# SandeepaInduwaraSamaranayake/SwinVox

Hardware: AMD Instinct MI355X
Metric: views/sec fwd+bwd SwinVox-T 224^2, 32^3 voxel, n_views=8 (higher is better)
Workload: dtype bf16; 1 GPU; SwinVox-T full pipeline (ResNet50[:layer3] || Swin multi-stage, cross-view attention, decoder, merger, refiner), fwd+2xBCE+bwd, train mode, B=64 samples x V=8 views of 224x224 per GPU; global_batch=64, n_views=8, images_per_gpu=512, parallelism=single GPU, launch=eager (one host launch per kernel, three streams)

## Files before the change

### include/swinvox_hip.h

```cpp
#ifndef SWINVOX_HIP_H
#define SWINVOX_HIP_H
#include <stddef.h>
#include <stdint.h>

#ifdef __cplusplus
extern "C" {
#endif

#define SV_OK 0
#define SV_ERR_INVALID (-1)
#define SV_ERR_LAUNCH (-2)

enum { SV_ACT_NONE = 0, SV_ACT_RELU = 1, SV_ACT_GELU = 2, SV_ACT_LRELU = 3 };
#define SV_BN_SLOTS 16
enum { SV_MATH_F32 = 0, SV_MATH_BF16 = 1, SV_MATH_FP8 = 2, SV_MATH_FP8_FULL = 3 };
enum { SV_F32 = 0, SV_BF16 = 1 };

const char* sv_last_error(void);
int sv_version(void);

typedef struct sv_geom {
  int N;
  int Di, Hi, Wi;
  int Do, Ho, Wo;
  int Ci, Co;
  int kd, kh, kw;
  int sd, sh, sw;
  int pd, ph, pw;
  int ldi;
} sv_geom;

typedef struct sv_epilogue {
  const float* bias;
  const void* residual;
  int ldr;
  const float* row_scale;
  int rows_per_scale;
  void* pre_act;
  double* stats;
  int act;
  float slope;
  const void* act_grad_src;
  int act_grad_kind;
  int ldc;
  int col_off;
} sv_epilogue;

int sv_conv_gather(const void* in, const void* w_packed, void* out, const sv_geom* g, const sv_epilogue* e,
                   int math, int act_dtype, void* stream);
int sv_set_conv_halo(int mode);
int sv_conv_halo_mode(void);
int sv_set_conv_halo_wgrad(int mode);
long long sv_conv_halo_launches(void);
int sv_conv_gather_is_wide(const void* in, const void* w, void* out, const sv_geom* g, const sv_epilogue* e, int math, int act_dtype);
int sv_tconv_gather(const void* in, const void* w_packed, void* out, const sv_geom* g, const sv_epilogue* e,
                    int math, int act_dtype, void* stream);
int sv_conv_wgrad_is_wide(const void* anchor, int lda, const void* gathered, const sv_geom* g, int cg_valid, int math, int act_dtype);
size_t sv_conv_wgrad_workspace_floats(const sv_geom* g);
int sv_conv_wgrad(const void* anchor, int lda, const void* gathered, float* dw, const sv_geom* g, int cg_valid,
                  float* workspace, float* dbias , int math, int act_dtype,
                  void* stream);
int sv_quant_rows_e4m3(const void* src, int src_dtype, int rows, int K, int ld, void* dst_q, int Kp, float* scales, void* stream);
int sv_linear_fp8(const void* xq, const float* sx, const void* wq, const float* sw, void* out, int M, int K, int N, const sv_epilogue* e,
                  int act_dtype, void* stream);
int sv_linear_fp8_supported(int K, int N, const sv_epilogue* e, int math, int act_dtype);
long long sv_linear_fp8_launches(void);
int sv_quant_cols_e4m3(const void* src, int src_dtype, int M, int C, int ld, void* dst_q, int Mp, float* scales, float* colsum, void* stream);
int sv_linear_fp8_dgrad(const void* dq, const float* sd, const void* wtq, const float* swt, void* dx, int M, int N, int K, const sv_epilogue* e,
                        int act_dtype, void* stream);
int sv_linear_fp8_dgrad_supported(int N, int K, const sv_epilogue* e, int math, int act_dtype);
int sv_linear_fp8_wgrad(const void* dyt, const float* sdc, const void* xt, const float* sxc, float* dw, int M, int N, int K, int ldw, int splits,
                        void* stream);
long long sv_linear_fp8_bwd_launches(int which);
int sv_stencil3_fwd(const void* x, int ldx, int cin_load, int groups, const void* w_bf16, int ntiles16,
                    const float* bias, void* out, int ldc, int col_off, int cout, const void* residual, int ldr,
                    double* stats, int I, int D, int H, int W, long long x_plane_stride, long long out_plane_stride, int act_dtype,
                    void* stream);
size_t sv_stencil3_wgrad_workspace_floats(int cout, int cin);
int sv_stencil3_wgrad(const void* x, int ldx, int cin_load, int groups, const void* dy, int lddy, int cout_load,
                      float* dw, float* dbias, float* workspace, int cout, int cin, int c_stride, int c_valid, int I, int D, int H, int W,
                      long long x_plane_stride, int act_dtype, void* stream);
int sv_tconv4s2_fwd(const void* x, const void* w_packed, const float* bias, void* out, double* stats, int I, int D, int H, int W,
                    int cin, int cout, void* stream);
int sv_pack_weight(const float* src, void* dst, int A, int B, int T, int swap, int pad_to, int out_dtype, void* stream);
typedef struct sv_pack_desc {
  const float* src; void* dst;
  int A, B, T, swap, rows_out, inner_out, block0, reserved;
} sv_pack_desc;
int sv_pack_weights_block_elems(void);
int sv_pack_weights(const sv_pack_desc* descs_dev, int n, int total_blocks, int out_dtype, void* stream);
int sv_colsum(const void* x, int rows, int cols, int ld, float* out, int accumulate, int act_dtype, void* stream);
int sv_cast(const void* src, int src_dtype, void* dst, int dst_dtype, long long n, void* stream);

int sv_layernorm_fwd(const void* x, const float* gamma, const float* beta, void* y, float* mean, float* rstd,
                     long long rows, int C, float eps, int merge_H, int merge_W, int act_dtype, void* stream);
size_t sv_layernorm_bwd_workspace_floats(int C);
int sv_layernorm_bwd(const void* dy, const void* x, const float* gamma, const float* mean, const float* rstd,
                     void* dx, float* dgamma, float* dbeta, float* workspace, long long rows, int C, int merge_H, int merge_W,
                     int accumulate_dx, int act_dtype, void* stream);
size_t sv_ln_image_workspace_floats(int I, int L);
int sv_ln_image_fwd(const void* x, const float* w, const float* b, void* y, float* meanrstd, float* workspace,
                    int I, int L, float eps, float drop_p, uint32_t seed, const uint32_t* seed_epoch, int act_dtype, void* stream);
int sv_ln_image_bwd(const void* dy, const void* x, const float* w, const float* meanrstd, void* dx, float* dw,
                    float* db, double* sums_ws , int I, int L, float drop_p, uint32_t seed,
                    const uint32_t* seed_epoch, int act_dtype, void* stream);
int sv_bn_stats(const void* x, long long M, int C, int ld, double* sums, int act_dtype, void* stream);
int sv_bn_finalize(const double* sums, long long count, const float* gamma, const float* beta, float* running_mean,
                   float* running_var, float momentum, float eps, int training, float* scale, float* shift,
                   float* save_mean, float* save_rstd, int C, void* stream);
int sv_scale_shift_act(const void* x, int ldx, const float* scale, const float* shift, const void* residual, int ldr,
                       void* y, int ldy, long long M, int C, int act, float slope, int act_dtype, void* stream);
int sv_bn_act_maxpool_fwd(const void* x, const float* scale, const float* shift, void* pooled, void* idx, int N, int H, int W, int C,
                          int act, float slope, int act_dtype, void* stream);
int sv_bn_maxpool_bwd(const void* dpooled, const void* idx, const void* x, const float* gamma, const float* save_mean, const float* save_rstd,
                      const float* fwd_scale, const float* fwd_shift, int N, int H, int W, int C, int act, float slope, int training,
                      void* dx, float* dgamma, float* dbeta, double* sums_ws, int act_dtype, void* stream);
int sv_bn_act_maxpool3d_fwd(const void* x, const float* scale, const float* shift, void* pooled, void* idx, int N, int D, int H, int W, int C,
                            int act, float slope, int act_dtype, void* stream);
int sv_bn_maxpool3d_bwd(const void* dpooled, const void* idx, const void* x, const float* gamma, const float* save_mean, const float* save_rstd,
                        const float* fwd_scale, const float* fwd_shift, int N, int D, int H, int W, int C, int act, float slope, int training,
                        void* dx, float* dgamma, float* dbeta, double* sums_ws, int act_dtype, void* stream);
size_t sv_bn_bwd_workspace_doubles(int C);
int sv_bn_bwd(const void* dz, int lddz, const void* z, int ldz, const void* x, int ldx, const float* gamma,
              const float* save_mean, const float* save_rstd, long long M, int C, int act, float slope, int training,
              void* dx, int lddx, void* dres, int lddres, float* dgamma, float* dbeta, double* sums_ws ,
              const float* fwd_scale, const float* fwd_shift ,
              int act_dtype, void* stream);
int sv_bn_signs_supported(int C);
int sv_scale_shift_act_signs(const void* x, int ldx, const float* scale, const float* shift, const void* residual, int ldr, void* y, int ldy,
                             long long M, int C, int act, float slope, void* signs, int act_dtype, void* stream);
int sv_bn_bwd_signs(const void* dz, int lddz, const void* signs, const void* x, int ldx, const float* gamma, const float* save_mean,
                    const float* save_rstd, long long M, int C, int act, float slope, int training, void* dx, int lddx, void* dres, int lddres,
                    float* dgamma, float* dbeta, double* sums_ws, int act_dtype, void* stream);

int sv_window_attention_fwd(const void* qkv, const float* table, void* out, int I, int H, int W, int C, int heads,
                            int shift, int math, int act_dtype, void* stream);
size_t sv_window_attention_bwd_workspace_floats(int heads);
int sv_window_attention_bwd(const void* qkv, const float* table, const void* dout, void* dqkv, float* dtable, float* workspace,
                            int I, int H, int W, int C, int heads, int shift, int math, int act_dtype, void* stream);
int sv_window_attention_windows_per_group(int I, int H, int W, int heads, int math, int backward);
int sv_cross_view_attention_fwd(const void* qkv, void* out, int B, int V, int P, int R, int heads, int act_dtype, void* stream);
int sv_cross_view_attention_bwd(const void* qkv, const void* dout, void* dqkv, int B, int V, int P, int R, int heads,
                                int act_dtype, void* stream);

int sv_transpose(const void* src, void* dst, int batch, int R, int C, int lds, int ldd, long long src_bstride,
                 long long dst_bstride, int act_dtype, void* stream);
int sv_add_n(const void* a, const void* b, const void* c, const void* d, void* out, long long M, int C, int ldo, int act_dtype, void* stream);
int sv_axpby(const void* a, const void* b, void* out, float alpha, float beta, long long n, int act_dtype, void* stream);
int sv_relu_bwd(const void* dy, const void* y, void* out, long long n, int act_dtype, void* stream);
int sv_maxpool2d_fwd(const void* x, void* y, uint8_t* idx, int N, int H, int W, int C, int act_dtype, void* stream);
int sv_maxpool2d_bwd(const void* dy, const uint8_t* idx, void* dx, int N, int H, int W, int C, int act_dtype, void* stream);
int sv_avgpool2_fwd(const void* x, void* y, int N, int H, int W, int C, int ldy, int col_off, int act_dtype, void* stream);
int sv_avgpool2_bwd(const void* dy, void* dx, int N, int H, int W, int C, int ldy, int col_off, int act_dtype, void* stream);
int sv_decoder_seed_fwd(const void* feat, void* out, int I, int C, int act_dtype, void* stream);
int sv_decoder_seed_bwd(const void* dout, void* dfeat, int I, int C, int act_dtype, void* stream);
int sv_maxpool3d_fwd(const void* x, void* y, uint8_t* idx, int N, int D, int H, int W, int C, int act_dtype, void* stream);
int sv_maxpool3d_bwd(const void* dy, const uint8_t* idx, void* dx, int N, int D, int H, int W, int C, int act_dtype, void* stream);
int sv_dropout(const void* x, void* y, long long n, float p, uint32_t seed, const uint32_t* seed_epoch, int act_dtype, void* stream);
int sv_droppath_scale(float* scale, int I, float p, uint32_t seed, const uint32_t* seed_epoch, void* stream);
int sv_rowscale(const void* x, const float* scale, void* y, long long rows, int C, int rows_per_scale, int act_dtype, void* stream);
int sv_dwconv2x2_fwd(const void* x, const float* w, const float* b, void* y, int I, int C, int act_dtype, void* stream);
int sv_dwconv2x2_bwd(const void* dy, const void* x, const float* w, void* dx, float* dw, float* db, int I, int C, int act_dtype, void* stream);
int sv_upsample3to7_add_fwd(const void* small, const void* x, int ldx, void* y, int I, int C, int act_dtype, void* stream);
int sv_upsample3to7_bwd(const void* dy, void* dsmall, int I, int C, int act_dtype, void* stream);
int sv_cva_downsample_fwd(const void* x, const float* w, const float* b, void* y, int I, int C, int r, int act_dtype, void* stream);
int sv_cva_downsample_bwd(const void* dy, const void* x, const float* w, void* dx, float* dw, float* db, int I, int C, int r, int act_dtype, void* stream);
int sv_cva_upsample_add_fwd(const void* small, const void* x, int ldx, void* y, int I, int C, int r, int act_dtype, void* stream);
int sv_cva_upsample_bwd(const void* dy, void* dsmall, int I, int C, int r, int act_dtype, void* stream);
int sv_decoder_head_fwd(const void* x8, const float* w, const float* bias, void* raw12, void* vol, long long M, int act_dtype, void* stream);
int sv_decoder_head_bwd(const void* draw12, const void* dvol, const void* x8, const float* w, void* dx8, float* dw, float* dbias,
                        long long M, int act_dtype, void* stream);
int sv_merge_views_fwd(const void* wlogit, const void* vol, void* out, int B, int V, int S, int act_dtype, void* stream);
int sv_merge_views_bwd(const void* wlogit, const void* vol, const void* out, const void* dout, void* dwlogit, void* dvol,
                       int B, int V, int S, int act_dtype, void* stream);
int sv_swin_mlp_supported(int C);
int sv_swin_mlp_pack(const float* w1, const float* w2, void* packs, int C, void* stream);
int sv_swin_mlp_fwd(const void* x1, void* x2, const float* ln_g, const float* ln_b, const void* packs, const float* b1, const float* b2,
                    const float* row_scale, int rows_per_scale, long long M, int C, float eps, void* stream);
int sv_swin_mlp_bwd(const void* x1, const void* dx2, void* dx1, const float* ln_g, const float* ln_b, const void* packs, const float* b1,
                    const float* row_scale, int rows_per_scale, float* dgamma, float* dbeta, long long M, int C, float eps, void* stream);
int sv_swin_mlp_wgrad(const void* x1, const void* dx2, const float* ln_g, const float* ln_b, const void* w1_rows, const void* w2t_rows,
                      const float* b1, const float* row_scale, int rows_per_scale, float* dw1, float* db1, float* dw2, float* db2,
                      long long M, int C, float eps, void* stream);

int sv_swin_attn_block_supported(int C, int heads, int act_dtype, int math);
int sv_swin_attn_block_fwd(const void* x, const float* ln_g, const float* ln_b, const float* wqkv, const float* bqkv, const float* table,
                           const float* wproj, const float* bproj, const float* row_scale, void* x1, void* ln1, float* mean, float* rstd,
                           void* qkv, void* att, int I, int H, int W, int C, int heads, int shift, float eps, int act_dtype, void* stream);
int sv_swin_attn_block_windows_per_group(int I, int H, int W, int backward);
int sv_swin_attn_block_bwd(const void* dx1, const void* qkv, const void* x, const float* mean, const float* rstd, const float* ln_g,
                           const float* wqkv, const float* wproj, const float* table, const float* row_scale, void* dqkv, void* dx,
                           void* dbr, float* dgamma, float* dbeta, float* dtable, float* workspace, int I, int H, int W, int C,
                           int heads, int shift, int act_dtype, void* stream);

int sv_encoder_prep(const void* images, int images_f32, void* x16, void* xp, int I, int S, int act_dtype, void* stream);
int sv_encoder_prep_bwd(const void* dx16, const void* dxp, void* dimages, int out_f32, int I, int S, int act_dtype, void* stream);
int sv_head_pack_x(const void* x, void* xc, int N, int D, int act_dtype, void* stream);
int sv_head_unpack_dx(const void* dxc, void* dx, int N, int D, int act_dtype, void* stream);
int sv_stem_space_to_depth(const void* images, void* x16, int I, int act_dtype, void* stream);
int sv_stem_pack(const float* w, void* wp, int out_dtype, void* stream);
int sv_stem_unpack_grad(const float* dw16, float* dw, void* stream);
int sv_stem_native(const float* w, float* w16, void* stream);
int sv_merger_pack(const float* w, void* wp_bf16, int cout, int cin, int dgrad, int concat, void* stream);

int sv_mean_views(const float* vol, float* out, int B, int V, int S, void* stream);
int sv_bce_logits(const float* x, const float* t, long long n, float* loss_accum, float* dx, const float* gscale_dev, void* stream);
int sv_iou_counts(const float* logits, const float* gt, const float* thresholds_dev, int nth, int B, int S, float* counts, void* stream);

int sv_grad_sumsq(const float* g, long long n, float gscale, double* slots16, void* stream);
int sv_adam_step(float* p, const float* g, float* m, float* v, long long n, double lr, double beta1, double beta2, double eps,
                 double weight_decay, long long step, float gscale, const double* slots16, float max_norm,
                 long long* skipped_steps, void* stream);
int sv_sgd_step(float* p, const float* g, float* momentum_buf, long long n, double lr, double momentum, double weight_decay,
// ... 20 lines not shown
```

### swinvox_amd/csrc/common.h

```cpp
#pragma once
#include <hip/hip_runtime.h>
#include <stdint.h>
#include <stdio.h>
#include "../../include/swinvox_hip.h"

namespace sv {

typedef float f32x4 __attribute__((ext_vector_type(4)));
typedef __bf16 bf16x8 __attribute__((ext_vector_type(8)));
typedef __bf16 bf16x4 __attribute__((ext_vector_type(4)));

template <typename T> __device__ __forceinline__ float ldf(const T* p) { return (float)*p; }
template <typename T> __device__ __forceinline__ void stf(T* p, float v) { *p = (T)v; }
__device__ __forceinline__ float4 ld4f(const float* p) { return *reinterpret_cast<const float4*>(p); }
__device__ __forceinline__ float4 ld4f(const __bf16* p) {
  const bf16x4 b = *reinterpret_cast<const bf16x4*>(p);
  return make_float4((float)b[0], (float)b[1], (float)b[2], (float)b[3]);
}
__device__ __forceinline__ void st4f(float* p, float4 v) { *reinterpret_cast<float4*>(p) = v; }
__device__ __forceinline__ void st4f(__bf16* p, float4 v) {
  bf16x4 b;
  b[0] = (__bf16)v.x; b[1] = (__bf16)v.y; b[2] = (__bf16)v.z; b[3] = (__bf16)v.w;
  *reinterpret_cast<bf16x4*>(p) = b;
}
// ... 94 lines not shown
  __syncthreads();
  if ((threadIdx.x & 63) == 0) scratch[w] = v;
  __syncthreads();
  float r = 0.f;
#pragma unroll
  for (int i = 0; i < NW; ++i) r += scratch[i];
  return r;
}

__device__ __forceinline__ float gelu_erf(float x) { return 0.5f * x * (1.f + erff(x * 0.70710678118654752440f)); }
__device__ __forceinline__ float gelu_erf_grad(float x) {
  const float cdf = 0.5f * (1.f + erff(x * 0.70710678118654752440f));
  const float pdf = 0.39894228040143267794f * expf(-0.5f * x * x);
  return cdf + x * pdf;
}

__device__ __forceinline__ float gelu_fast(float x) {
  const float x2 = fminf(x * x, 64.f);
  const float p = fmaf(x2, fmaf(x2, 9.975397e-04f, -1.0665937e-01f), -2.3012706e+00f);
  return x * __builtin_amdgcn_rcpf(1.f + __builtin_amdgcn_exp2f(x * p));
}
__device__ __forceinline__ float gelu_grad_fast(float x) {
  const float x2 = fminf(x * x, 64.f);
  const float p = fmaf(x2, fmaf(x2, 9.975397e-04f, -1.0665937e-01f), -2.3012706e+00f);
  const float s = __builtin_amdgcn_rcpf(1.f + __builtin_amdgcn_exp2f(x * p));
  const float qd = fmaf(x2, fmaf(x2, -3.45720919e-03f, 2.21791923e-01f), 1.59511919f);
  return s * fmaf(x * (1.f - s), qd, 1.f);
}
typedef float f32x2 __attribute__((ext_vector_type(2)));
__device__ __forceinline__ f32x2 gelu_sigma2(f32x2 x, f32x2& x2) {
  x2 = x * x;
  x2[0] = fminf(x2[0], 64.f); x2[1] = fminf(x2[1], 64.f);
  const f32x2 p = __builtin_elementwise_fma(x2, __builtin_elementwise_fma(x2, (f32x2)(9.975397e-04f), (f32x2)(-1.0665937e-01f)), (f32x2)(-2.3012706e+00f));
  const f32x2 xp = x * p;
  f32x2 e;
  e[0] = __builtin_amdgcn_exp2f(xp[0]); e[1] = __builtin_amdgcn_exp2f(xp[1]);
  e = e + (f32x2)(1.f);
  f32x2 s;
  s[0] = __builtin_amdgcn_rcpf(e[0]); s[1] = __builtin_amdgcn_rcpf(e[1]);
  return s;
}
__device__ __forceinline__ f32x2 gelu_fast2(f32x2 x) { f32x2 x2; return x * gelu_sigma2(x, x2); }
__device__ __forceinline__ void gelu_both_fast2(f32x2 x, f32x2& g, f32x2& dg) {
  f32x2 x2;
  const f32x2 s = gelu_sigma2(x, x2);
  const f32x2 qd = __builtin_elementwise_fma(x2, __builtin_elementwise_fma(x2, (f32x2)(-3.45720919e-03f), (f32x2)(2.21791923e-01f)), (f32x2)(1.59511919f));
  g = x * s;
  dg = s * __builtin_elementwise_fma(x * ((f32x2)(1.f) - s), qd, (f32x2)(1.f));
}
__device__ __forceinline__ f32x2 gelu_grad_fast2(f32x2 x) { f32x2 g, dg; gelu_both_fast2(x, g, dg); return dg; }
template <bool FAST> __device__ __forceinline__ float gelu_t(float x) {
  if constexpr (FAST) return gelu_fast(x);
  else return gelu_erf(x);
}
template <bool FAST> __device__ __forceinline__ float gelu_grad_t(float x) {
  if constexpr (FAST) return gelu_grad_fast(x);
  else return gelu_erf_grad(x);
}
template <bool FAST> __device__ __forceinline__ float apply_act_t(float v, int act, float slope) {
  switch (act) {
    case SV_ACT_RELU: return v > 0.f ? v : 0.f;
    case SV_ACT_GELU: return gelu_t<FAST>(v);
    case SV_ACT_LRELU: return v > 0.f ? v : v * slope;
    default: return v;
  }
}
template <bool FAST> __device__ __forceinline__ float act_grad_t(float pre, int act, float slope) {
  switch (act) {
    case SV_ACT_RELU: return pre > 0.f ? 1.f : 0.f;
    case SV_ACT_GELU: return gelu_grad_t<FAST>(pre);
    case SV_ACT_LRELU: return pre > 0.f ? 1.f : slope;
    default: return 1.f;
  }
}

__device__ __forceinline__ float apply_act(float v, int act, float slope) {
  switch (act) {
    case SV_ACT_RELU: return v > 0.f ? v : 0.f;
    case SV_ACT_GELU: return gelu_erf(v);
    case SV_ACT_LRELU: return v > 0.f ? v : v * slope;
    default: return v;
  }
}
__device__ __forceinline__ float act_grad(float pre, int act, float slope) {
  switch (act) {
    case SV_ACT_RELU: return pre > 0.f ? 1.f : 0.f;
    case SV_ACT_GELU: return gelu_erf_grad(pre);
    case SV_ACT_LRELU: return pre > 0.f ? 1.f : slope;
    default: return 1.f;
  }
}

__device__ __forceinline__ uint32_t hash_u32(uint32_t seed, uint32_t idx_lo, uint32_t idx_hi) {
  uint32_t x = seed ^ (idx_lo * 0x9E3779B1u) ^ (idx_hi * 0x85EBCA77u);
  x ^= x >> 16; x *= 0x7FEB352Du; x ^= x >> 15; x *= 0x846CA68Bu; x ^= x >> 16;
  x += idx_lo; x ^= x >> 13; x *= 0xC2B2AE35u; x ^= x >> 16;
  return x;
}
__device__ __forceinline__ uint32_t eff_seed(uint32_t seed, const uint32_t* epoch) {
  return epoch ? seed + epoch[0] * 0x9E3779B1u : seed;
}
__device__ __forceinline__ float uniform01(uint32_t seed, uint64_t idx) {
  return (hash_u32(seed, (uint32_t)idx, (uint32_t)(idx >> 32)) >> 8) * (1.0f / 16777216.0f);
}

}
```

### swinvox_amd/csrc/norm.hip

```cpp
#include "common.h"
#include <stdlib.h>

namespace sv {

constexpr int BN_BWD_SLOTS = 16, LN_BWD_SLOTS = 32;

struct MergeMap { int H, W, C0; };

template <bool MERGE>
__device__ __forceinline__ size_t ln_src_off(long long row, int e, int C, const MergeMap& mm) {
  if constexpr (!MERGE) return (size_t)row * C + e;
  const int blk = e / mm.C0, c = e - blk * mm.C0;
  const int wp = blk >> 1, hp = blk & 1;
  const int W2 = mm.W >> 1, H2 = mm.H >> 1;
  const int x2 = (int)(row % W2); long long t = row / W2;
  const int y2 = (int)(t % H2); const long long i = t / H2;
  return ((size_t)(i * mm.H + 2 * y2 + hp) * mm.W + (2 * x2 + wp)) * mm.C0 + c;
}

template <int VEC, typename AT> struct LnIO;
template <typename AT> struct LnIO<4, AT> {
  static __device__ __forceinline__ void load(const AT* p, float* v) { const float4 q = ld4f(p); v[0] = q.x; v[1] = q.y; v[2] = q.z; v[3] = q.w; }
  static __device__ __forceinline__ void store(AT* p, const float* v) { st4f(p, make_float4(v[0], v[1], v[2], v[3])); }
};
// ... 529 lines not shown
        float zz[4];
        if (z) { const float4 zv = ld4f(z + (size_t)r * ldz + 4 * g); zz[0] = zv.x; zz[1] = zv.y; zz[2] = zv.z; zz[3] = zv.w; }
        else {
#pragma unroll
          for (int j = 0; j < 4; ++j) zz[j] = __fmaf_rn(xx[j], msc[j], msh[j]);
        }
#pragma unroll
        for (int j = 0; j < 4; ++j) d[j] *= zz[j] > 0.f ? 1.f : neg;
      }
#pragma unroll
      for (int j = 0; j < 4; ++j) { s1[j] += d[j]; s2[j] += d[j] * (xx[j] - mu[j]) * rs[j]; }
    }
  }
  for (int gg = 0; gg < 4; ++gg) {
    __syncthreads();
    if (g == gg) {
#pragma unroll
      for (int j = 0; j < 4; ++j) { red[rl][j] = (double)s1[j]; red[rl][4 + j] = (double)s2[j]; }
    }
    __syncthreads();
    if (threadIdx.x < 8) {
      const int c = 4 * gg + (threadIdx.x & 3);
      if (c < C) {
        double a = 0.0;
        for (int l = 0; l < 64; ++l) a += red[l][threadIdx.x];
        atomicAdd(sums + (size_t)(blockIdx.x % BN_BWD_SLOTS) * 2 * C + (threadIdx.x >> 2) * C + c, a);
      }
    }
  }
}

template <typename AT>
__global__ __launch_bounds__(256) void bn_bwd_apply_narrow_kernel(const AT* __restrict__ dz, int lddz, const AT* __restrict__ z, int ldz,
                                                                  const AT* __restrict__ x, int ldx, const float* __restrict__ gamma,
                                                                  const float* __restrict__ mean, const float* __restrict__ rstd,
                                                                  const double* __restrict__ sums, long long M, int C, int act, float slope,
                                                                  int training, AT* __restrict__ dx, int lddx, AT* __restrict__ dres, int lddres,
                                                                  const float* __restrict__ fsc, const float* __restrict__ fsh) {
  sums += (size_t)BN_BWD_SLOTS * 2 * C;
  const int g = threadIdx.x & 3, rl = threadIdx.x >> 2;
  if (4 * g >= C) return;
  float msc[4], msh[4];
#pragma unroll
  for (int j = 0; j < 4; ++j) { const int c = 4 * g + j; msc[j] = (!z && fsc && c < C) ? fsc[c] : 0.f; msh[j] = (!z && fsh && c < C) ? fsh[c] : 0.f; }
  double k1[4], k2[4], k3[4];
  const double invM = 1.0 / (double)M;
#pragma unroll
  for (int j = 0; j < 4; ++j) {
    const int c = 4 * g + j;
    if (c < C) {
      const double gm = gamma[c], rs = rstd[c], mu = mean[c];
      k1[j] = gm * rs;
      if (training) { const double a = sums[c] * invM, b = sums[C + c] * invM; k3[j] = gm * rs * b * rs; k2[j] = gm * rs * a - k3[j] * mu; }
      else { k2[j] = 0.0; k3[j] = 0.0; }
    } else { k1[j] = k2[j] = k3[j] = 0.0; }
  }
  const float neg = act == SV_ACT_LRELU ? slope : 0.f;
  for (long long r = (long long)blockIdx.x * 64 + rl; r < M; r += (long long)gridDim.x * 64) {
    const float4 dv = ld4f(dz + (size_t)r * lddz + 4 * g), xv = ld4f(x + (size_t)r * ldx + 4 * g);
    float d[4] = {dv.x, dv.y, dv.z, dv.w};
    const float xx[4] = {xv.x, xv.y, xv.z, xv.w};
    if (act != SV_ACT_NONE) {
      float zz[4];
      if (z) { const float4 zv = ld4f(z + (size_t)r * ldz + 4 * g); zz[0] = zv.x; zz[1] = zv.y; zz[2] = zv.z; zz[3] = zv.w; }
      else {
#pragma unroll
        for (int j = 0; j < 4; ++j) zz[j] = __fmaf_rn(xx[j], msc[j], msh[j]);
      }
#pragma unroll
      for (int j = 0; j < 4; ++j) d[j] *= zz[j] > 0.f ? 1.f : neg;
    }
    float o[4];
#pragma unroll
    for (int j = 0; j < 4; ++j) {
      const bool real = 4 * g + j < C;
      o[j] = real ? (float)(k1[j] * (double)d[j] - k2[j] - k3[j] * (double)xx[j]) : 0.f;
      if (!real) d[j] = 0.f;
    }
    if (dres) st4f(dres + (size_t)r * lddres + 4 * g, make_float4(d[0], d[1], d[2], d[3]));
    st4f(dx + (size_t)r * lddx + 4 * g, make_float4(o[0], o[1], o[2], o[3]));
  }
}

template <typename AT>
__global__ __launch_bounds__(256) void scale_shift_act_cg_kernel(const AT* __restrict__ x, int ldx, const float* __restrict__ scale,
                                                                 const float* __restrict__ shift, const AT* __restrict__ res, int ldr,
                                                                 AT* __restrict__ y, int ldy, long long M, int C, int act, float slope,
                                                                 long long rows_per_block, int G, unsigned long long* __restrict__ signs) {
  const int gq = threadIdx.x % G, rl = threadIdx.x / G, RL = 256 / G;
  const int c = (blockIdx.x * G + gq) * 4;
  if (c >= C || rl >= RL) return;
  const float4 sc = *reinterpret_cast<const float4*>(scale + c), sh = *reinterpret_cast<const float4*>(shift + c);
  const long long r0 = (long long)blockIdx.y * rows_per_block;
  long long r1 = r0 + rows_per_block; if (r1 > M) r1 = M;
#pragma unroll 2
  for (long long r = r0 + rl; r < r1; r += RL) {
    const float4 xv = ld4f(x + (size_t)r * ldx + c);
    float o[4] = {__fmaf_rn(xv.x, sc.x, sh.x), __fmaf_rn(xv.y, sc.y, sh.y), __fmaf_rn(xv.z, sc.z, sh.z), __fmaf_rn(xv.w, sc.w, sh.w)};
    if (res) {
      const float4 rv = ld4f(res + (size_t)r * ldr + c);
      o[0] += rv.x; o[1] += rv.y; o[2] += rv.z; o[3] += rv.w;
    }
    if (signs) {
      const unsigned long long b0 = __builtin_amdgcn_ballot_w64(o[0] > 0.f), b1 = __builtin_amdgcn_ballot_w64(o[1] > 0.f);
      const unsigned long long b2 = __builtin_amdgcn_ballot_w64(o[2] > 0.f), b3 = __builtin_amdgcn_ballot_w64(o[3] > 0.f);
      if (gq == 0) {
        unsigned long long* w = signs + ((size_t)r * (C >> 8) + blockIdx.x) * 4;
        *reinterpret_cast<ulonglong2*>(w) = make_ulonglong2(b0, b1);
        *reinterpret_cast<ulonglong2*>(w + 2) = make_ulonglong2(b2, b3);
      }
    }
#pragma unroll
    for (int j = 0; j < 4; ++j) o[j] = apply_act(o[j], act, slope);
    st4f(y + (size_t)r * ldy + c, make_float4(o[0], o[1], o[2], o[3]));
  }
}

template <typename AT>
__global__ __launch_bounds__(256) void bn_bwd_apply_cg_kernel(const AT* __restrict__ dz, int lddz, const AT* __restrict__ z, int ldz,
                                                              const AT* __restrict__ x, int ldx, const float* __restrict__ gamma,
                                                              const float* __restrict__ mean, const float* __restrict__ rstd,
                                                              const double* __restrict__ sums, long long M, int C, int act, float slope,
                                                              int training, AT* __restrict__ dx, int lddx, AT* __restrict__ dres, int lddres,
                                                              const float* __restrict__ fsc, const float* __restrict__ fsh,
                                                              long long rows_per_block, int G) {
  const int gq = threadIdx.x % G, rl = threadIdx.x / G, RL = 256 / G;
  const int c = (blockIdx.x * G + gq) * 4;
  if (c >= C || rl >= RL) return;
  sums += (size_t)BN_BWD_SLOTS * 2 * C;
  double k1[4], k2[4], k3[4];
  const double invM = 1.0 / (double)M;
  float msc[4] = {0.f, 0.f, 0.f, 0.f}, msh[4] = {0.f, 0.f, 0.f, 0.f};
#pragma unroll
  for (int j = 0; j < 4; ++j) {
    const double gm = gamma[c + j], rs = rstd[c + j], mu = mean[c + j];
    k1[j] = gm * rs;
    if (training) { const double a = sums[c + j] * invM, b = sums[C + c + j] * invM; k3[j] = gm * rs * b * rs; k2[j] = gm * rs * a - k3[j] * mu; }
    else { k2[j] = 0.0; k3[j] = 0.0; }
    if (!z && act != SV_ACT_NONE) { msc[j] = fsc[c + j]; msh[j] = fsh[c + j]; }
  }
  const float neg = act == SV_ACT_LRELU ? slope : 0.f;
  const long long r0 = (long long)blockIdx.y * rows_per_block;
  long long r1 = r0 + rows_per_block; if (r1 > M) r1 = M;
#pragma unroll 2
  for (long long r = r0 + rl; r < r1; r += RL) {
    const float4 dv = ld4f(dz + (size_t)r * lddz + c), xv = ld4f(x + (size_t)r * ldx + c);
    float d[4] = {dv.x, dv.y, dv.z, dv.w};
    const float xx[4] = {xv.x, xv.y, xv.z, xv.w};
    if (act != SV_ACT_NONE) {
      float zz[4];
      if (z) { const float4 zv = ld4f(z + (size_t)r * ldz + c); zz[0] = zv.x; zz[1] = zv.y; zz[2] = zv.z; zz[3] = zv.w; }
      else {
#pragma unroll
        for (int j = 0; j < 4; ++j) zz[j] = __fmaf_rn(xx[j], msc[j], msh[j]);
      }
#pragma unroll
      for (int j = 0; j < 4; ++j) d[j] *= zz[j] > 0.f ? 1.f : neg;
    }
    if (dres) st4f(dres + (size_t)r * lddres + c, make_float4(d[0], d[1], d[2], d[3]));
    float o[4];
#pragma unroll
    for (int j = 0; j < 4; ++j) o[j] = (float)(k1[j] * (double)d[j] - k2[j] - k3[j] * (double)xx[j]);
    st4f(dx + (size_t)r * lddx + c, make_float4(o[0], o[1], o[2], o[3]));
  }
}

template <typename AT>
__global__ __launch_bounds__(256) void bn_bwd_reduce_vec_kernel(const AT* __restrict__ dz, int lddz, const AT* __restrict__ z, int ldz,
                                                                const AT* __restrict__ x, int ldx, const float* __restrict__ mean,
                                                                const float* __restrict__ rstd, long long M, int C, int act, float slope,
                                                                double* __restrict__ sums, long long rows_per_block, int G,
                                                                const float* __restrict__ fsc, const float* __restrict__ fsh,
                                                                AT* __restrict__ dmask, int lddm, const unsigned long long* __restrict__ signs) {
  __shared__ double red[256][9];
  const int gq = threadIdx.x % G, rl = threadIdx.x / G, RL = 256 / G;
  const int c = (blockIdx.x * G + gq) * 4;
  const long long r0 = (long long)blockIdx.y * rows_per_block;
  long long r1e = r0 + rows_per_block; if (r1e > M) r1e = M;
  double s1[4] = {0.0, 0.0, 0.0, 0.0}, s2[4] = {0.0, 0.0, 0.0, 0.0};
  if (c < C && rl < RL) {
    const float4 mu = *reinterpret_cast<const float4*>(mean + c), rs = *reinterpret_cast<const float4*>(rstd + c);
    float4 msc = make_float4(0.f, 0.f, 0.f, 0.f), msh = msc;
    if (!z && !signs && act != SV_ACT_NONE) { msc = *reinterpret_cast<const float4*>(fsc + c); msh = *reinterpret_cast<const float4*>(fsh + c); }
// ... 413 lines not shown
  SV_REQUIRE_ACT(act_dtype);
  SV_REQUIRE(((uintptr_t)gamma & 15) == 0, "layernorm_bwd: gamma must be 16-byte aligned");
  hipStream_t s = (hipStream_t)stream;
  MergeMap mm{merge_H, merge_W, merge_H > 0 ? C / 4 : 0};
  const bool v8 = ln_vec8(act_dtype, C, merge_H, dy, x, dx);
  if (merge_H > 0) {
    if (v8) ln_bwd_launch<true, __bf16, 8>(dy, x, gamma, mean, rstd, dx, dgamma, dbeta, rows, C, mm, accumulate_dx, workspace, s);
    else if (act_dtype == SV_BF16) ln_bwd_launch<true, __bf16, 4>(dy, x, gamma, mean, rstd, dx, dgamma, dbeta, rows, C, mm, accumulate_dx, workspace, s);
    else ln_bwd_launch<true, float, 4>(dy, x, gamma, mean, rstd, dx, dgamma, dbeta, rows, C, mm, accumulate_dx, workspace, s);
  } else {
    if (v8) ln_bwd_launch<false, __bf16, 8>(dy, x, gamma, mean, rstd, dx, dgamma, dbeta, rows, C, mm, accumulate_dx, workspace, s);
    else if (act_dtype == SV_BF16) ln_bwd_launch<false, __bf16, 4>(dy, x, gamma, mean, rstd, dx, dgamma, dbeta, rows, C, mm, accumulate_dx, workspace, s);
    else ln_bwd_launch<false, float, 4>(dy, x, gamma, mean, rstd, dx, dgamma, dbeta, rows, C, mm, accumulate_dx, workspace, s);
  }
  return check_launch("sv_layernorm_bwd");
}

static inline int lnl_image_slices(int I, int L) {
  int s = 2048 / cdiv(L, 1024);
  if (s > I / 8) s = I / 8;
  return s < 1 ? 1 : (s > 32 ? 32 : s);
}

extern "C" size_t sv_ln_image_workspace_floats(int I, int L) { return (size_t)I * cdiv(L, LNL_CHUNK) * 2; }

extern "C" int sv_ln_image_fwd(const void* x, const float* w, const float* b, void* y, float* meanrstd, float* workspace,
                               int I, int L, float eps, float drop_p, uint32_t seed, const uint32_t* seed_epoch, int act_dtype, void* stream) {
  SV_REQUIRE(x && w && b && y && meanrstd && workspace && I > 0 && L > 0 && L % 4 == 0, "ln_image_fwd: bad arguments (I=%d L=%d)", I, L);
  SV_REQUIRE_ACT(act_dtype);
  hipStream_t s = (hipStream_t)stream;
  const int nch = cdiv(L, LNL_CHUNK);
  int gx = cdiv(L, 1024); if (gx > 64) gx = 64;
  SV_DISPATCH_ACT(act_dtype,
    hipLaunchKernelGGL(lnl_moments_kernel<AT>, dim3(nch, I), dim3(256), 0, s, static_cast<const AT*>(x), workspace, L, nch);
    hipLaunchKernelGGL(lnl_finalize_kernel, dim3(cdiv(I, 64)), dim3(64), 0, s, workspace, meanrstd, L, nch, eps, I);
    hipLaunchKernelGGL(lnl_apply_kernel<AT>, dim3(gx, I), dim3(256), 0, s, static_cast<const AT*>(x), w, b, meanrstd, static_cast<AT*>(y), L, drop_p, seed, seed_epoch););
  return check_launch("sv_ln_image_fwd");
}

extern "C" int sv_ln_image_bwd(const void* dy, const void* x, const float* w, const float* meanrstd, void* dx, float* dw,
                               float* db, double* sums_ws, int I, int L, float drop_p, uint32_t seed, const uint32_t* seed_epoch, int act_dtype, void* stream) {
  SV_REQUIRE(dy && x && w && meanrstd && dx && dw && db && sums_ws && I > 0 && L > 0 && L % 4 == 0, "ln_image_bwd: bad arguments");
  SV_REQUIRE_ACT(act_dtype);
  hipStream_t s = (hipStream_t)stream;
  (void)hipMemsetAsync(sums_ws, 0, sizeof(double) * 2 * I, s);
  int gx = cdiv(L, 1024); if (gx > 32) gx = 32;
  SV_DISPATCH_ACT(act_dtype,
    hipLaunchKernelGGL(lnl_bwd_reduce_kernel<AT>, dim3(gx, I), dim3(256), 0, s, static_cast<const AT*>(dy), static_cast<const AT*>(x), w, meanrstd, sums_ws, L, drop_p, seed, seed_epoch);
    hipLaunchKernelGGL(lnl_bwd_apply_kernel<AT>, dim3(cdiv(L, 1024), lnl_image_slices(I, L)), dim3(256), 0, s, static_cast<const AT*>(dy), static_cast<const AT*>(x), w, meanrstd, sums_ws,
                       static_cast<AT*>(dx), dw, db, L, I, drop_p, seed, seed_epoch););
  return check_launch("sv_ln_image_bwd");
}

extern "C" int sv_bn_stats(const void* x, long long M, int C, int ld, double* sums, int act_dtype, void* stream) {
  SV_REQUIRE(x && sums && M > 0 && C > 0 && ld >= C, "bn_stats: bad arguments");
  SV_REQUIRE_ACT(act_dtype);
  const int cg = cdiv(C, 64);
  long long splits = 2048 / cg; if (splits < 1) splits = 1;
  const long long maxs = (M + 63) / 64; if (splits > maxs) splits = maxs;
  const long long rpb = (M + splits - 1) / splits;
  SV_DISPATCH_ACT(act_dtype, hipLaunchKernelGGL(bn_stats_kernel<AT>, dim3(cg, cdiv(M, rpb)), dim3(256), 0, (hipStream_t)stream, static_cast<const AT*>(x), M, C, ld, sums, rpb););
  return check_launch("sv_bn_stats");
}

extern "C" int sv_bn_finalize(const double* sums, long long count, const float* gamma, const float* beta, float* running_mean,
                              float* running_var, float momentum, float eps, int training, float* scale, float* shift,
                              float* save_mean, float* save_rstd, int C, void* stream) {
  SV_REQUIRE(gamma && beta && running_mean && running_var && scale && shift && save_mean && save_rstd && C > 0, "bn_finalize: null argument");
  SV_REQUIRE(!training || (sums && count > 0), "bn_finalize: training needs sums and a positive count");
  hipLaunchKernelGGL(bn_finalize_kernel, dim3(cdiv(C, 64)), dim3(64), 0, (hipStream_t)stream, sums, (double)count, gamma, beta,
                     running_mean, running_var, momentum, eps, training, scale, shift, save_mean, save_rstd, C);
  return check_launch("sv_bn_finalize");
}

static inline bool aligned4(int act_dtype, const void* a, const void* b = nullptr, const void* c = nullptr, const void* d = nullptr,
                            const void* e = nullptr) {
  const uintptr_t m = act_dtype == SV_BF16 ? 7 : 15;
  return (((uintptr_t)a | (uintptr_t)b | (uintptr_t)c | (uintptr_t)d | (uintptr_t)e) & m) == 0;
}

static inline bool bn_signs_ok(int C) { return C % 256 == 0; }

static int scale_shift_act_impl(const void* x, int ldx, const float* scale, const float* shift, const void* residual, int ldr,
                                void* y, int ldy, long long M, int C, int act, float slope, unsigned long long* signs, int act_dtype, void* stream) {
  SV_REQUIRE(x && scale && shift && y && M > 0 && C > 0 && ldx >= C && ldy >= C, "scale_shift_act: bad arguments");
  SV_REQUIRE_ACT(act_dtype);
  hipStream_t s = (hipStream_t)stream;
  const bool vec = (C % 4 == 0) && (ldx % 4 == 0) && (ldy % 4 == 0) && (!residual || ldr % 4 == 0) && aligned4(act_dtype, x, y, residual) &&
                   (((uintptr_t)scale | (uintptr_t)shift) & 15) == 0;
  const bool narrow = !vec && C <= BN_NARROW_MAXC && (ldx % 4 == 0) && (ldy % 4 == 0) && ldx >= ((C + 3) & ~3) && ldy >= ((C + 3) & ~3) &&
                      (!residual || (ldr % 4 == 0 && ldr >= ((C + 3) & ~3))) && aligned4(act_dtype, x, y, residual);
  SV_REQUIRE(!signs || (vec && bn_signs_ok(C) && ((uintptr_t)signs & 15) == 0), "scale_shift_act_signs: needs C %% 256 == 0 and 4-aligned rows (C=%d)", C);
  if (narrow) {
    long long blocks = (M + 63) / 64; if (blocks > 8192) blocks = 8192;
    SV_DISPATCH_ACT(act_dtype, hipLaunchKernelGGL(scale_shift_act_narrow_kernel<AT>, dim3((unsigned)blocks), dim3(256), 0, s, static_cast<const AT*>(x), ldx, scale, shift,
                                                  static_cast<const AT*>(residual), ldr, static_cast<AT*>(y), ldy, M, C, act, slope););
  } else if (vec) {
    const int G = C / 4 < 64 ? C / 4 : 64, RL = 256 / G;
    const int cg = cdiv(C / 4, G);
    long long splits = 4096 / cg; if (splits < 1) splits = 1;
    const long long maxs = (M + 4 * RL - 1) / (4 * RL); if (splits > maxs) splits = maxs;
    const long long rpb = (M + splits - 1) / splits;
    SV_DISPATCH_ACT(act_dtype, hipLaunchKernelGGL(scale_shift_act_cg_kernel<AT>, dim3(cg, cdiv(M, rpb)), dim3(256), 0, s, static_cast<const AT*>(x), ldx, scale, shift,
                                                  static_cast<const AT*>(residual), ldr, static_cast<AT*>(y), ldy, M, C, act, slope, rpb, G, signs););
  } else {
    long long blocks = (M * C + 255) / 256; if (blocks > 8192) blocks = 8192;
    SV_DISPATCH_ACT(act_dtype, hipLaunchKernelGGL(scale_shift_act_scalar_kernel<AT>, dim3((unsigned)blocks), dim3(256), 0, s, static_cast<const AT*>(x), ldx, scale, shift,
                                                  static_cast<const AT*>(residual), ldr, static_cast<AT*>(y), ldy, M, C, act, slope););
  }
  return check_launch("sv_scale_shift_act");
}

extern "C" int sv_scale_shift_act(const void* x, int ldx, const float* scale, const float* shift, const void* residual, int ldr,
                                  void* y, int ldy, long long M, int C, int act, float slope, int act_dtype, void* stream) {
  return scale_shift_act_impl(x, ldx, scale, shift, residual, ldr, y, ldy, M, C, act, slope, nullptr, act_dtype, stream);
}
extern "C" int sv_bn_signs_supported(int C) { return bn_signs_ok(C) ? 1 : 0; }
extern "C" int sv_scale_shift_act_signs(const void* x, int ldx, const float* scale, const float* shift, const void* residual, int ldr,
                                        void* y, int ldy, long long M, int C, int act, float slope, void* signs, int act_dtype, void* stream) {
  SV_REQUIRE(signs, "scale_shift_act_signs: null sign buffer");
  return scale_shift_act_impl(x, ldx, scale, shift, residual, ldr, y, ldy, M, C, act, slope, static_cast<unsigned long long*>(signs), act_dtype, stream);
}

static bool bn_pool_shape_ok(int N, int H, int W, int C) {
  return N > 0 && H > 0 && W > 0 && C > 0 && C % 4 == 0 && C <= 1024 && 256 % (C / 4) == 0 && (long long)N * H * W * C < (1ll << 40);
}
static bool bn_pool_cv8(int act_dtype, int C, const void* a, const void* b, const void* c) {
  return act_dtype == SV_BF16 && C % 8 == 0 && 256 % (C / 8) == 0 && (((uintptr_t)a | (uintptr_t)b | (uintptr_t)c) & 15) == 0;
}
extern "C" int sv_bn_act_maxpool_fwd(const void* x, const float* scale, const float* shift, void* pooled, void* idx, int N, int H, int W, int C,
                                     int act, float slope, int act_dtype, void* stream) {
  SV_REQUIRE(x && scale && shift && pooled && idx && bn_pool_shape_ok(N, H, W, C), "bn_act_maxpool_fwd: bad arguments (N=%d H=%d W=%d C=%d)", N, H, W, C);
  SV_REQUIRE_ACT(act_dtype);
  SV_REQUIRE(aligned4(act_dtype, x, pooled, nullptr, nullptr, nullptr) && (((uintptr_t)scale | (uintptr_t)shift) & 15) == 0 && ((uintptr_t)idx & 3) == 0,
             "bn_act_maxpool_fwd: misaligned buffers");
  const int Ho = (H + 1) / 2, Wo = (W + 1) / 2;
  const long long total = (long long)N * Ho * Wo * (C / 4);
  long long blocks = (total + 255) / 256; if (blocks > 16384) blocks = 16384;
  if (bn_pool_cv8(act_dtype, C, x, pooled, idx)) {
    const long long t8 = total / 2;
    long long b8 = (t8 + 255) / 256; if (b8 > 16384) b8 = 16384;
    hipLaunchKernelGGL((bn_act_maxpool_fwd_kernel<__bf16, 8>), dim3((unsigned)b8), dim3(256), 0, (hipStream_t)stream, static_cast<const __bf16*>(x),
                       scale, shift, static_cast<__bf16*>(pooled), static_cast<uint8_t*>(idx), N, H, W, C, Ho, Wo, act, slope);
    return check_launch("sv_bn_act_maxpool_fwd");
  }
  SV_DISPATCH_ACT(act_dtype, hipLaunchKernelGGL((bn_act_maxpool_fwd_kernel<AT, 4>), dim3((unsigned)blocks), dim3(256), 0, (hipStream_t)stream, static_cast<const AT*>(x),
                                                scale, shift, static_cast<AT*>(pooled), static_cast<uint8_t*>(idx), N, H, W, C, Ho, Wo, act, slope););
  return check_launch("sv_bn_act_maxpool_fwd");
}
extern "C" int sv_bn_maxpool_bwd(const void* dpooled, const void* idx, const void* x, const float* gamma, const float* save_mean, const float* save_rstd,
                                 const float* fwd_scale, const float* fwd_shift, int N, int H, int W, int C, int act, float slope, int training,
                                 void* dx, float* dgamma, float* dbeta, double* sums_ws, int act_dtype, void* stream) {
  SV_REQUIRE(dpooled && idx && x && gamma && save_mean && save_rstd && fwd_scale && fwd_shift && dx && dgamma && dbeta && sums_ws && bn_pool_shape_ok(N, H, W, C),
             "bn_maxpool_bwd: bad arguments (N=%d H=%d W=%d C=%d)", N, H, W, C);
  SV_REQUIRE_ACT(act_dtype);
  SV_REQUIRE(aligned4(act_dtype, dpooled, x, dx, nullptr, nullptr) && (((uintptr_t)save_mean | (uintptr_t)save_rstd | (uintptr_t)fwd_scale | (uintptr_t)fwd_shift) & 15) == 0 &&
             ((uintptr_t)idx & 3) == 0, "bn_maxpool_bwd: misaligned buffers");
  hipStream_t s = (hipStream_t)stream;
  const int Ho = (H + 1) / 2, Wo = (W + 1) / 2;
  const long long rows = (long long)N * Ho;
  SV_REQUIRE(rows < (1ll << 31), "bn_maxpool_bwd: more than 2^31 image rows");
  int rpb = (int)((rows + 2047) / 2048); if (rpb < 1) rpb = 1;
  const unsigned nb = (unsigned)((rows + rpb - 1) / rpb);
  int rpa = (int)((rows + 8191) / 8192); if (rpa < 1) rpa = 1;
  const unsigned na = (unsigned)((rows + rpa - 1) / rpa);
  if (bn_pool_cv8(act_dtype, C, dpooled, x, dx) && ((uintptr_t)idx & 7) == 0) {
    typedef __bf16 AT;
    hipLaunchKernelGGL((bn_pool_bwd_reduce_kernel<AT, 8>), dim3(nb), dim3(256), 0, s, static_cast<const AT*>(dpooled), static_cast<const uint8_t*>(idx), static_cast<const AT*>(x),
                       save_mean, save_rstd, fwd_scale, fwd_shift, sums_ws, N, H, W, C, Ho, Wo, act, slope, rpb);
    hipLaunchKernelGGL(bn_bwd_fold_kernel, dim3(cdiv(2 * C, 256)), dim3(256), 0, s, sums_ws, C, dgamma, dbeta);
    hipLaunchKernelGGL((bn_pool_bwd_apply_kernel<AT, 8>), dim3(na), dim3(256), 0, s, static_cast<const AT*>(dpooled), static_cast<const uint8_t*>(idx), static_cast<const AT*>(x),
                       gamma, save_mean, save_rstd, fwd_scale, fwd_shift, sums_ws, static_cast<AT*>(dx), N, H, W, C, Ho, Wo, act, slope, training, rpa);
    return check_launch("sv_bn_maxpool_bwd");
  }
  SV_DISPATCH_ACT(act_dtype,
    hipLaunchKernelGGL((bn_pool_bwd_reduce_kernel<AT, 4>), dim3(nb), dim3(256), 0, s, static_cast<const AT*>(dpooled), static_cast<const uint8_t*>(idx), static_cast<const AT*>(x),
                       save_mean, save_rstd, fwd_scale, fwd_shift, sums_ws, N, H, W, C, Ho, Wo, act, slope, rpb);
    hipLaunchKernelGGL(bn_bwd_fold_kernel, dim3(cdiv(2 * C, 256)), dim3(256), 0, s, sums_ws, C, dgamma, dbeta);
    hipLaunchKernelGGL((bn_pool_bwd_apply_kernel<AT, 4>), dim3(na), dim3(256), 0, s, static_cast<const AT*>(dpooled), static_cast<const uint8_t*>(idx), static_cast<const AT*>(x),
                       gamma, save_mean, save_rstd, fwd_scale, fwd_shift, sums_ws, static_cast<AT*>(dx), N, H, W, C, Ho, Wo, act, slope, training, rpa););
  return check_launch("sv_bn_maxpool_bwd");
}

extern "C" int sv_bn_act_maxpool3d_fwd(const void* x, const float* scale, const float* shift, void* pooled, void* idx, int N, int D, int H, int W, int C,
                                       int act, float slope, int act_dtype, void* stream) {
  SV_REQUIRE(x && scale && shift && pooled && idx && D > 1 && bn_pool_shape_ok(N, H, W, C) && (long long)N * D * H * W * C < (1ll << 40),
             "bn_act_maxpool3d_fwd: bad arguments (N=%d D=%d H=%d W=%d C=%d)", N, D, H, W, C);
  SV_REQUIRE_ACT(act_dtype);
  SV_REQUIRE(aligned4(act_dtype, x, pooled, nullptr, nullptr, nullptr) && ((uintptr_t)idx & 3) == 0, "bn_act_maxpool3d_fwd: misaligned buffers");
  const long long win = (long long)N * (D / 2) * (H / 2) * (W / 2);
  if (win == 0) return SV_OK;
  hipStream_t s = (hipStream_t)stream;
  if (bn_pool_cv8(act_dtype, C, x, pooled, idx)) {
    long long blocks = (win * (C / 8) + 255) / 256; if (blocks > 16384) blocks = 16384;
    hipLaunchKernelGGL((bn_act_maxpool3d_fwd_kernel<__bf16, 8>), dim3((unsigned)blocks), dim3(256), 0, s, static_cast<const __bf16*>(x), scale, shift,
                       static_cast<__bf16*>(pooled), static_cast<uint8_t*>(idx), N, D, H, W, C, act, slope);
  } else {
    long long blocks = (win * (C / 4) + 255) / 256; if (blocks > 16384) blocks = 16384;
    SV_DISPATCH_ACT(act_dtype, hipLaunchKernelGGL((bn_act_maxpool3d_fwd_kernel<AT, 4>), dim3((unsigned)blocks), dim3(256), 0, s, static_cast<const AT*>(x), scale, shift,
                                                  static_cast<AT*>(pooled), static_cast<uint8_t*>(idx), N, D, H, W, C, act, slope););
  }
  return check_launch("sv_bn_act_maxpool3d_fwd");
}
extern "C" int sv_bn_maxpool3d_bwd(const void* dpooled, const void* idx, const void* x, const float* gamma, const float* save_mean, const float* save_rstd,
// ... 104 lines not shown
```

### swinvox_amd/csrc/stencil.hip

```cpp
#include "common.h"
#include <map>
#include <mutex>
#include <type_traits>

namespace sv {

constexpr int TZ = 4, TY = 8, TX = 8;
constexpr int HZ = TZ + 2, HY = TY + 2, HX = TX + 2;
constexpr int HPOS = HZ * HY * HX;
constexpr int NVOX = TZ * TY * TX;
typedef __attribute__((address_space(3))) bf16x4 lds_bf16x4_t;

__device__ __forceinline__ bf16x4 to_bf16x4(float4 v) {
  bf16x4 b;
  b[0] = (__bf16)v.x; b[1] = (__bf16)v.y; b[2] = (__bf16)v.z; b[3] = (__bf16)v.w;
  return b;
}
__device__ __forceinline__ bf16x4 to_bf16x4(bf16x4 v) { return v; }

__device__ __forceinline__ int xcd_first_tile() {
  const int n = gridDim.x, b = blockIdx.x;
  return (n & 7) == 0 ? (b & 7) * (n >> 3) + (b >> 3) : b;
}

struct TileId { int img, z0, y0, x0; };
template <int TZV = TZ>
__device__ __forceinline__ TileId tile_of(int t, int D, int H, int W) {
  const int tz = D / TZV, ty = H / TY, tx = W / TX;
  TileId r;
  r.x0 = (t % tx) * TX; t /= tx; r.y0 = (t % ty) * TY; t /= ty; r.z0 = (t % tz) * TZV; r.img = t / tz;
  return r;
}

template <int G, typename AT, int TZV = TZ, int NTHR = 256>
struct HaloRegs {
  static constexpr int HZV = TZV + 2, HPOSV = HZV * HY * HX;
  static constexpr int C = 16 * G, VPP = C / 4, N = (HPOSV * VPP + NTHR - 1) / NTHR;
  typedef typename std::conditional<G == 1, int, long long>::type OffT;
  typename V4<AT>::type r[N];
  OffT off[N];
  int face[N];
  int lds[N];
  __device__ __forceinline__ void init(int ldx, long long plane, int cin_load, int H, int W, int tid, int pitch = HX) {
#pragma unroll
    for (int k = 0; k < N; ++k) {
      const int i = tid + NTHR * k;
      const int h = i / VPP, v = i - h * VPP;
      const int hx = h % HX; const int t2 = h / HX; const int hy = t2 % HY; const int hz = t2 / HY;
      const int cv = v * 4, pl = plane ? cv / ldx : 0;
      face[k] = (hz == 0 ? 1 : 0) | (hz == HZV - 1 ? 2 : 0) | (hy == 0 ? 4 : 0) | (hy == HY - 1 ? 8 : 0) | (hx == 0 ? 16 : 0) | (hx == HX - 1 ? 32 : 0) |
                ((i < HPOSV * VPP && cv < cin_load) ? 0 : 64);
      off[k] = (OffT)pl * (OffT)plane + (OffT)(((hz * H + hy) * W + hx) * ldx + (cv - pl * ldx));
      lds[k] = ((hz * HY + hy) * pitch + hx) * C + cv;
    }
  }
  __device__ __forceinline__ void load(const AT* __restrict__ x, int ldx, const TileId& t, int D, int H, int W) {
    const int out = (t.z0 == 0 ? 1 : 0) | (t.z0 + TZV == D ? 2 : 0) | (t.y0 == 0 ? 4 : 0) | (t.y0 + TY == H ? 8 : 0) | (t.x0 == 0 ? 16 : 0) | (t.x0 + TX == W ? 32 : 0) | 64;
    const AT* corner = x + ((((long long)t.img * D + t.z0 - 1) * H + t.y0 - 1) * W + t.x0 - 1) * (long long)ldx;
#pragma unroll
    for (int k = 0; k < N; ++k) {
      typename V4<AT>::type q = V4<AT>::zero();
#ifndef SV_ST_PROBE_NOLOAD
      if ((face[k] & out) == 0) q = V4<AT>::load(corner + off[k]);
#endif
      r[k] = q;
    }
  }
  __device__ __forceinline__ void store(__bf16* Xs, int tid) const {
#pragma unroll
    for (int k = 0; k < N; ++k) {
      const int i = tid + NTHR * k;
      if (i < HPOSV * VPP) *reinterpret_cast<bf16x4*>(Xs + lds[k]) = to_bf16x4(r[k]);
    }
  }
};

template <typename AT>
struct StencilArgsT {
  const AT* x; int ldx; int cin_load;
  long long x_plane, out_plane;
  const __bf16* w;
  const float* bias; AT* out; int ldc; int col_off; int cout;
  const AT* residual; int ldr;
  double* stats;
  int I, D, H, W, ntiles;
};

template <int G> struct StencilPitch { static constexpr int HXP = G == 1 ? 16 : HX; };
template <int G> struct StencilBrick { static constexpr int TZV = 8, NTHR = TZV * 64; };
template <int G> struct StencilBrickF { static constexpr int TZV = 8, NTHR = TZV * 64; };
template <int G, int NT, typename AT, bool VEC>
__global__ __launch_bounds__(StencilBrickF<G>::NTHR, 2) void stencil3_fwd_kernel(const StencilArgsT<AT> p) {
  constexpr int C = 16 * G, KTOT = 27 * C, KPAD = (KTOT + 31) / 32 * 32, NSTEP = KPAD / 32, HXP = StencilPitch<G>::HXP;
  constexpr int TZV = StencilBrickF<G>::TZV, NTHR = StencilBrickF<G>::NTHR, NW = NTHR / 64;
  __shared__ __attribute__((aligned(16))) char xc[(TZV + 2) * HY * HXP * C * 2];
  __shared__ __attribute__((aligned(16))) __bf16 Ws[NT * 16 * KPAD];
  __shared__ float red[16 * 16 * 2];
  __bf16* Xs = reinterpret_cast<__bf16*>(xc);
  const int tid = threadIdx.x, lane = tid & 63, wave = tid >> 6;
  const int lr = lane & 15, lg = lane >> 4;

  for (int i = tid; i < NT * 16 * KPAD / 8; i += NTHR) {
    const int n = (i * 8) / KPAD, k = (i * 8) - n * KPAD;
    bf16x8 v = VecN<__bf16, 8>::zero();
    if (k < KTOT) v = *reinterpret_cast<const bf16x8*>(p.w + (size_t)n * KTOT + k);
    *reinterpret_cast<bf16x8*>(Ws + n * KPAD + k) = v;
  }
  const int cs4 = (p.cout + 3) & ~3;
  float bias4[NT][4], st1[4] = {0.f, 0.f, 0.f, 0.f}, st2[4] = {0.f, 0.f, 0.f, 0.f};
#pragma unroll
  for (int nt = 0; nt < NT; ++nt)
#pragma unroll
    for (int j = 0; j < 4; ++j) { const int n = nt * 16 + lg * 4 + j; bias4[nt][j] = (p.bias && n < p.cout) ? p.bias[n] : 0.f; }

  HaloRegs<G, AT, TZV, NTHR> hr;
  hr.init(p.ldx, p.x_plane, p.cin_load, p.H, p.W, tid, HXP);
  int tile = xcd_first_tile();
  TileId t = tile_of<TZV>(tile < p.ntiles ? tile : 0, p.D, p.H, p.W);
  if (tile < p.ntiles) { hr.load(p.x, p.ldx, t, p.D, p.H, p.W); hr.store(Xs, tid); }
  __syncthreads();
  const int yy = lr >> 3, xx = lr & 7;
  int toff[NSTEP];
#pragma unroll
  for (int s = 0; s < NSTEP; ++s) {
    const int kb = s * 32 + lg * 8;
    int tap = kb / C; const int c = kb - tap * C;
    if (tap > 26) tap = 26;
    const int dz = tap / 9, dy = (tap - dz * 9) / 3, dx = tap - dz * 9 - dy * 3;
    toff[s] = (((dz * HY + dy) * HXP + dx) * C + c) * 2;
  }
  const char* xrow = xc + ((wave * HY + yy) * HXP + xx) * C * 2;
  const char* wrow = reinterpret_cast<const char*>(Ws) + (lr * KPAD + lg * 8) * 2;
  const int n0 = lg * 4;
  bool colreal[NT][4];
#pragma unroll
  for (int nt = 0; nt < NT; ++nt)
#pragma unroll
    for (int j = 0; j < 4; ++j) colreal[nt][j] = nt * 16 + n0 + j < p.cout;
  for (; tile < p.ntiles; tile += gridDim.x) {
    const int next = tile + gridDim.x;
    TileId tn = t;
    if (next < p.ntiles) { tn = tile_of<TZV>(next, p.D, p.H, p.W); hr.load(p.x, p.ldx, tn, p.D, p.H, p.W); }

    f32x4 acc[4][NT];
#pragma unroll
    for (int mt = 0; mt < 4; ++mt)
#pragma unroll
      for (int nt = 0; nt < NT; ++nt) acc[mt][nt] = (f32x4){0.f, 0.f, 0.f, 0.f};
#ifndef SV_ST_PROBE_NOMMA
#pragma unroll
    for (int s = 0; s < NSTEP; ++s) {
      bf16x8 b[NT];
#pragma unroll
      for (int nt = 0; nt < NT; ++nt) b[nt] = *reinterpret_cast<const bf16x8*>(wrow + nt * 16 * KPAD * 2 + s * 64);
      const char* ap = xrow + toff[s];
#pragma unroll
      for (int mt = 0; mt < 4; ++mt) {
        const bf16x8 a = *reinterpret_cast<const bf16x8*>(ap + mt * (2 * HXP * C * 2));
#pragma unroll
        for (int nt = 0; nt < NT; ++nt) acc[mt][nt] = __builtin_amdgcn_mfma_f32_16x16x32_bf16(b[nt], a, acc[mt][nt], 0, 0, 0);
      }
    }
#endif
    const size_t pos0 = (((size_t)t.img * p.D + t.z0 + wave) * p.H + t.y0 + yy) * p.W + t.x0 + xx;
    if constexpr (VEC) {
#pragma unroll
      for (int nt = 0; nt < NT; ++nt) {
        const int nn = nt * 16 + n0;
        if (nn >= cs4) continue;
        AT* orow; const AT* rrow = nullptr;
        if (p.out_plane) { const int pl = nn / p.ldc; orow = p.out + (size_t)pl * p.out_plane + pos0 * p.ldc + (nn - pl * p.ldc); }
        else orow = p.out + pos0 * p.ldc + p.col_off + nn;
        if (p.residual) rrow = p.residual + pos0 * p.ldr + nn;
#pragma unroll
        for (int mt = 0; mt < 4; ++mt) {
          float v[4];
#pragma unroll
          for (int j = 0; j < 4; ++j) v[j] = colreal[nt][j] ? acc[mt][nt][j] + bias4[nt][j] : 0.f;
          if (NT == 1 && p.stats) {
#pragma unroll
            for (int j = 0; j < 4; ++j) { st1[j] += v[j]; st2[j] += v[j] * v[j]; }
          }
          if (p.residual) {
            const float4 rv = ld4f(rrow + (size_t)mt * 2 * p.W * p.ldr);
            v[0] += rv.x; v[1] += rv.y; v[2] += rv.z; v[3] += rv.w;
          }
#ifdef SV_ST_PROBE_NOSTORE
          if (v[0] == 1234.5f)
#endif
          st4f(orow + (size_t)mt * 2 * p.W * p.ldc, make_float4(v[0], v[1], v[2], v[3]));
        }
      }
    } else {
#pragma unroll
      for (int mt = 0; mt < 4; ++mt) {
        const size_t pos = pos0 + (size_t)mt * 2 * p.W;
#pragma unroll
        for (int nt = 0; nt < NT; ++nt) {
          const int nn = nt * 16 + n0;
#pragma unroll
          for (int j = 0; j < 4; ++j) {
            if (nn + j < p.cout) {
              float r = acc[mt][nt][j] + bias4[nt][j];
              if (NT == 1 && p.stats) { st1[j] += r; st2[j] += r * r; }
              if (p.residual) r += ldf(p.residual + pos * p.ldr + nn + j);
              stf(p.out + pos * p.ldc + p.col_off + nn + j, r);
            }
          }
        }
      }
    }
    t = tn;
    __syncthreads();
    if (next < p.ntiles) hr.store(Xs, tid);
    __syncthreads();
  }
  if (NT == 1 && p.stats) {
#pragma unroll
    for (int j = 0; j < 4; ++j) {
      { st1[j] += dpp_move<0xB1>(st1[j]); st1[j] += dpp_move<0x4E>(st1[j]); st1[j] += dpp_move<0x141>(st1[j]); st1[j] += dpp_move<0x140>(st1[j]);
        st2[j] += dpp_move<0xB1>(st2[j]); st2[j] += dpp_move<0x4E>(st2[j]); st2[j] += dpp_move<0x141>(st2[j]); st2[j] += dpp_move<0x140>(st2[j]); }
    }
    if (lr == 0) {
#pragma unroll
      for (int j = 0; j < 4; ++j) { red[(wave * 16 + lg * 4 + j) * 2] = st1[j]; red[(wave * 16 + lg * 4 + j) * 2 + 1] = st2[j]; }
    }
    __syncthreads();
    if (tid < 16 && tid < p.cout) {
      float a = 0.f, b = 0.f;
#pragma unroll
      for (int w = 0; w < NW; ++w) { a += red[(w * 16 + tid) * 2]; b += red[(w * 16 + tid) * 2 + 1]; }
      double* st = p.stats + (size_t)(blockIdx.x % SV_BN_SLOTS) * 2 * p.cout;
      atomicAdd(st + tid, (double)a);
      atomicAdd(st + p.cout + tid, (double)b);
    }
  }
}

template <typename AT>
struct StencilWArgsT {
  const AT* x; int ldx; int cin_load;
  long long x_plane;
  const AT* dy; int lddy; int cout_load;
  float* dw;
  float* ws;
  float* dbias;
  int cout, cin;
  int c_stride, c_valid;
  int I, D, H, W, ntiles;
};

constexpr int WG_SLOTS = 16;
__global__ __launch_bounds__(256) void stencil_wgrad_fold_kernel(const float* __restrict__ ws, float* __restrict__ dw, int n) {
  const int i = blockIdx.x * 256 + threadIdx.x;
  if (i >= n) return;
  float a = 0.f;
#pragma unroll
  for (int sl = 0; sl < WG_SLOTS; ++sl) a += ws[(size_t)sl * n + i];
  dw[i] += a;
}

template <int G, typename AT>
__global__ __launch_bounds__(StencilBrick<G>::NTHR, 2) void stencil3_wgrad_kernel(const StencilWArgsT<AT> p) {
  constexpr int C = 16 * G, TZV = StencilBrick<G>::TZV, NTHR = StencilBrick<G>::NTHR, NW = NTHR / 64, NTAPW = (27 + NW - 1) / NW;
  constexpr int HPOSV = (TZV + 2) * HY * HX, NVOXV = TZV * TY * TX;
  __shared__ __attribute__((aligned(16))) __bf16 Xs[HPOSV * C];
  __shared__ __attribute__((aligned(16))) __bf16 Ds[NVOXV * 16];
  __shared__ float bred[NTHR / 16 * 16];
  const int tid = threadIdx.x, lane = tid & 63, wave = tid >> 6;
  const int lr = lane & 15, lg = lane >> 4, q = lr >> 2, pp = lr & 3;
  const int ntap = (27 - wave + NW - 1) / NW;
  f32x4 acc[NTAPW][G];
#pragma unroll
  for (int i = 0; i < NTAPW; ++i)
#pragma unroll
    for (int gg = 0; gg < G; ++gg) acc[i][gg] = (f32x4){0.f, 0.f, 0.f, 0.f};
  float bsum = 0.f;

  HaloRegs<G, AT, TZV, NTHR> hr;
  hr.init(p.ldx, p.x_plane, p.cin_load, p.H, p.W, tid);
  typename V4<AT>::type dr[4];
  auto load_dy = [&](const TileId& t) {
#pragma unroll
    for (int k = 0; k < 4; ++k) {
      const int i = tid + NTHR * k;
      const int v = i >> 2, c4 = i & 3;
      const int xx = v % TX; const int t2 = v / TX; const int yy = t2 % TY; const int zz = t2 / TY;
      typename V4<AT>::type qv = V4<AT>::zero();
      if (c4 * 4 < p.cout_load)
        qv = V4<AT>::load(p.dy + ((((size_t)t.img * p.D + t.z0 + zz) * p.H + t.y0 + yy) * p.W + t.x0 + xx) * (size_t)p.lddy + c4 * 4);
      dr[k] = qv;
    }
  };
  auto store_dy = [&]() {
#pragma unroll
    for (int k = 0; k < 4; ++k) *reinterpret_cast<bf16x4*>(Ds + (tid + NTHR * k) * 4) = to_bf16x4(dr[k]);
  };

  int tile = xcd_first_tile();
  if (tile < p.ntiles) {
    const TileId t = tile_of<TZV>(tile, p.D, p.H, p.W);
    hr.load(p.x, p.ldx, t, p.D, p.H, p.W); load_dy(t);
    hr.store(Xs, tid); store_dy();
  }
  __syncthreads();
  for (; tile < p.ntiles; tile += gridDim.x) {
    const int next = tile + gridDim.x;
    if (next < p.ntiles) {
      const TileId t = tile_of<TZV>(next, p.D, p.H, p.W);
      hr.load(p.x, p.ldx, t, p.D, p.H, p.W); load_dy(t);
    }
    if (p.dbias) {
      const int c = tid & 15, vg = tid >> 4;
#pragma unroll
      for (int k = 0; k < 16; ++k) bsum += (float)Ds[(vg * 16 + k) * 16 + c];
    }
#pragma unroll 1
    for (int ch = 0; ch < 2 * TZV; ++ch) {
      const int z = ch >> 1, yb = (ch & 1) * 4 + lg;
      const __bf16* asrc = Ds + (((z * TY + yb) * TX) + q) * 16 + pp * 4;
      const bf16x4 alo = __builtin_amdgcn_ds_read_tr16_b64_v4bf16((lds_bf16x4_t*)(asrc));
      const bf16x4 ahi = __builtin_amdgcn_ds_read_tr16_b64_v4bf16((lds_bf16x4_t*)(asrc + 4 * 16));
      const bf16x8 a = __builtin_shufflevector(alo, ahi, 0, 1, 2, 3, 4, 5, 6, 7);
#pragma unroll
      for (int i = 0; i < NTAPW; ++i) {
        if (i < ntap) {
          const int tap = wave + NW * i;
          const int dz = tap / 9, dy = (tap - dz * 9) / 3, dx = tap - dz * 9 - dy * 3;
          const int hb = ((z + dz) * HY + yb + dy) * HX + dx + q;
#pragma unroll
          for (int gg = 0; gg < G; ++gg) {
            const __bf16* bsrc = Xs + hb * C + gg * 16 + pp * 4;
            const bf16x4 blo = __builtin_amdgcn_ds_read_tr16_b64_v4bf16((lds_bf16x4_t*)(bsrc));
            const bf16x4 bhi = __builtin_amdgcn_ds_read_tr16_b64_v4bf16((lds_bf16x4_t*)(bsrc + 4 * C));
            const bf16x8 b = __builtin_shufflevector(blo, bhi, 0, 1, 2, 3, 4, 5, 6, 7);
            acc[i][gg] = __builtin_amdgcn_mfma_f32_16x16x32_bf16(a, b, acc[i][gg], 0, 0, 0);
          }
        }
      }
    }
    __syncthreads();
    if (next < p.ntiles) { hr.store(Xs, tid); store_dy(); }
    __syncthreads();
  }
  if (p.dbias) {
    bred[tid] = bsum;
    __syncthreads();
    if (tid < 16 && tid < p.cout) {
      float a = 0.f;
#pragma unroll
      for (int g2 = 0; g2 < NTHR / 16; ++g2) a += bred[g2 * 16 + tid];
      atomicAdd(p.dbias + tid, a);
    }
  }
  float* dst = p.ws ? p.ws + (size_t)(blockIdx.x % WG_SLOTS) * p.cout * p.cin * 27 : p.dw;
#pragma unroll
  for (int i = 0; i < NTAPW; ++i) {
    if (i < ntap) {
      const int tap = wave + NW * i;
#pragma unroll
      for (int gg = 0; gg < G; ++gg) {
        const int cm = gg * 16 + lr;
        const int grp = cm / p.c_stride, within = cm - grp * p.c_stride;
// ... 56 lines not shown
    __syncthreads();
    const int yy = lr >> 3, xx = lr & 7;
#pragma unroll 1
    for (int ci = 0; ci < 2; ++ci) {
      const int cls = 2 * wave + ci, az = cls >> 2, ay = (cls >> 1) & 1, ax = cls & 1;
      bf16x8 b[8];
#pragma unroll
      for (int tt = 0; tt < 8; ++tt) {
        b[tt] = VecN<__bf16, 8>::zero();
        if (lr < 8) b[tt] = *reinterpret_cast<const bf16x8*>(Ws + (cls * 8 + lr) * 256 + tt * 32 + lg * 8);
      }
#pragma unroll 2
      for (int g = 0; g < 8; ++g) {
        const int jz = g >> 1, jy = (g & 1) * 2 + yy;
        const int base = ((jz + az) * T4_HY + (jy + ay)) * T4_HX + (xx + ax);
        f32x4 acc = (f32x4){0.f, 0.f, 0.f, 0.f};
#pragma unroll
        for (int tt = 0; tt < 8; ++tt) {
          const int off = ((tt >> 2) * T4_HY + ((tt >> 1) & 1)) * T4_HX + (tt & 1);
          const bf16x8 a = *reinterpret_cast<const bf16x8*>(Xs + (base + off) * 32 + lg * 8);
          acc = __builtin_amdgcn_mfma_f32_16x16x32_bf16(b[tt], a, acc, 0, 0, 0);
        }
        if (lg < 2) {
          bf16x4 o;
#pragma unroll
          for (int j = 0; j < 4; ++j) o[j] = (__bf16)(acc[j] + bias4[j]);
          const int oz = 2 * jz + az, oy = 2 * jy + ay, ox = 2 * xx + ax;
          *reinterpret_cast<bf16x4*>(Os + ((oz * 8 + oy) * 16 + ox) * 8 + lg * 4) = o;
        }
      }
    }
    __syncthreads();
#pragma unroll
    for (int k = 0; k < 4; ++k) {
      const int v = tid + 256 * k;
      const int ox = v & 15, oy = (v >> 4) & 7, oz = v >> 7;
      const bf16x8 o = *reinterpret_cast<const bf16x8*>(Os + v * 8);
      const size_t pos = (((size_t)img * (2 * p.D) + 2 * z0 + oz) * (2 * p.H) + 2 * y0 + oy) * (2 * p.W) + 2 * x0 + ox;
      *reinterpret_cast<bf16x8*>(p.out + pos * 8) = o;
      if (p.stats) {
#pragma unroll
        for (int c = 0; c < 8; ++c) { const double f = (double)(float)o[c]; st1[c] += f; st2[c] += f * f; }
      }
    }
    __syncthreads();
  }
  if (p.stats) {
#pragma unroll
    for (int c = 0; c < 8; ++c) {
      float a = (float)st1[c], b2 = (float)st2[c];
      a = wave_sum(a); b2 = wave_sum(b2);
      if (lane == 0) { red[wave][c] = a; red[wave][8 + c] = b2; }
    }
    __syncthreads();
    if (tid < 16 && (tid & 7) < p.cout) {
      const float v = red[0][tid] + red[1][tid] + red[2][tid] + red[3][tid];
      double* st = p.stats + (size_t)(blockIdx.x % SV_BN_SLOTS) * 2 * p.cout;
      atomicAdd(st + (tid >> 3) * p.cout + (tid & 7), (double)v);
    }
  }
}

}

using namespace sv;

static int resident_per_cu(const void* kernel, int threads = 256) {
  static std::mutex mu;
  static std::map<const void*, int> cache;
  std::lock_guard<std::mutex> lk(mu);
  auto it = cache.find(kernel);
  if (it != cache.end()) return it->second;
  int n = 0;
  if (hipOccupancyMaxActiveBlocksPerMultiprocessor(&n, kernel, threads, 0) != hipSuccess || n < 1) { (void)hipGetLastError(); n = 1; }
  cache[kernel] = n;
  return n;
}

static int stencil_check(int I, int D, int H, int W) {
  SV_REQUIRE(I > 0 && D % 8 == 0 && H % TY == 0 && W % TX == 0, "stencil3: grid %dx%dx%d must be a multiple of the 8x8x8 brick", D, H, W);
  return SV_OK;
}

#define SV_STENCIL_LAUNCH(GG, NTT, VV)                                                                                     \
  do {                                                                                                                    \
    constexpr int nthr = StencilBrickF<GG>::NTHR;                                                                         \
    const int nt_ = I * (D / StencilBrickF<GG>::TZV) * (H / TY) * (W / TX);                                               \
    a.ntiles = nt_;                                                                                                       \
    const int resident = 256 * resident_per_cu((const void*)stencil3_fwd_kernel<GG, NTT, AT, VV>, nthr);                  \
    hipLaunchKernelGGL((stencil3_fwd_kernel<GG, NTT, AT, VV>), dim3(nt_ < resident ? nt_ : resident), dim3(nthr), 0, s, a); \
  } while (0)

extern "C" int sv_stencil3_fwd(const void* x, int ldx, int cin_load, int groups, const void* w_bf16, int ntiles16,
                               const float* bias, void* out, int ldc, int col_off, int cout, const void* residual, int ldr,
                               double* stats, int I, int D, int H, int W, long long x_plane_stride, long long out_plane_stride,
                               int act_dtype, void* stream) {
  SV_REQUIRE(x && w_bf16 && out, "stencil3_fwd: null argument");
  SV_REQUIRE(x_plane_stride >= 0 && out_plane_stride >= 0 && x_plane_stride % 4 == 0 && out_plane_stride % 4 == 0, "stencil3_fwd: bad plane strides");
  SV_REQUIRE(!out_plane_stride || (col_off == 0 && !residual && ldc % 4 == 0 && cout % ldc == 0),
             "stencil3_fwd: planar output needs col_off == 0, no residual and whole planes of ldc (multiple of 4) columns");
  SV_REQUIRE_ACT(act_dtype);
  if (int rc = stencil_check(I, D, H, W)) return rc;
    SV_REQUIRE(cin_load % 4 == 0 && cin_load <= 16 * groups && ldx % 4 == 0 && (x_plane_stride ? cin_load % ldx == 0 : ldx >= cin_load),
             "stencil3_fwd: bad input channels (cin_load=%d ldx=%d groups=%d)", cin_load, ldx, groups);
  SV_REQUIRE(cout > 0 && cout <= 16 * ntiles16 && (out_plane_stride || ldc >= col_off + cout), "stencil3_fwd: bad output window");
  SV_REQUIRE(!stats || ntiles16 == 1, "stencil3_fwd: statistics need a single 16-column tile");
  const uintptr_t amask = act_dtype == SV_BF16 ? 7 : 15;
  SV_REQUIRE(((uintptr_t)x & amask) == 0 && ((uintptr_t)w_bf16 & 15) == 0, "stencil3_fwd: operands must be aligned to 4 elements");
  SV_REQUIRE((ldc & 3) != 0 || (((uintptr_t)out | (uintptr_t)residual) & amask) == 0,
             "stencil3_fwd: out/residual must be aligned to 4 elements when ldc is a multiple of 4");
  const int ntiles = I * (D / TZ) * (H / TY) * (W / TX);
  hipStream_t s = (hipStream_t)stream;
  if (!((groups == 1 && ntiles16 == 1) || (groups == 3 && ntiles16 == 1) || (groups == 1 && ntiles16 == 3))) {
    set_error("stencil3_fwd: unsupported (groups=%d, ntiles16=%d)", groups, ntiles16);
    return SV_ERR_INVALID;
  }
  SV_DISPATCH_ACT(act_dtype,
    const int cs4 = (cout + 3) & ~3;
    const bool vec = out_plane_stride != 0 || ((ldc & 3) == 0 && (col_off & 3) == 0 && col_off + cs4 <= ldc && (!residual || ((ldr & 3) == 0 && cs4 <= ldr)));
    StencilArgsT<AT> a{static_cast<const AT*>(x), ldx, cin_load, x_plane_stride, out_plane_stride, (const __bf16*)w_bf16, bias, static_cast<AT*>(out), ldc, col_off, cout,
                       static_cast<const AT*>(residual), ldr, stats, I, D, H, W, ntiles};
    if (groups == 1 && ntiles16 == 1) { if (vec) SV_STENCIL_LAUNCH(1, 1, true); else SV_STENCIL_LAUNCH(1, 1, false); }
    else if (groups == 3) { if (vec) SV_STENCIL_LAUNCH(3, 1, true); else SV_STENCIL_LAUNCH(3, 1, false); }
    else { if (vec) SV_STENCIL_LAUNCH(1, 3, true); else SV_STENCIL_LAUNCH(1, 3, false); });
  return check_launch("sv_stencil3_fwd");
}

extern "C" size_t sv_stencil3_wgrad_workspace_floats(int cout, int cin) { return (size_t)WG_SLOTS * cout * cin * 27; }

extern "C" int sv_stencil3_wgrad(const void* x, int ldx, int cin_load, int groups, const void* dy, int lddy, int cout_load,
                                 float* dw, float* dbias, float* workspace, int cout, int cin, int c_stride, int c_valid, int I, int D, int H,
                                 int W, long long x_plane_stride, int act_dtype, void* stream) {
  SV_REQUIRE(x && dy && dw, "stencil3_wgrad: null argument");
  SV_REQUIRE(x_plane_stride >= 0 && x_plane_stride % 4 == 0 && (!x_plane_stride || cin_load % ldx == 0), "stencil3_wgrad: bad plane stride");
  SV_REQUIRE_ACT(act_dtype);
  if (int rc = stencil_check(I, D, H, W)) return rc;
  SV_REQUIRE(cin_load % 4 == 0 && cin_load <= 16 * groups && ldx % 4 == 0 && cout_load % 4 == 0 && cout_load <= 16 && lddy % 4 == 0,
             "stencil3_wgrad: bad channel layout");
  SV_REQUIRE(cout > 0 && cout <= 16 && cin > 0 && c_stride > 0 && c_valid > 0, "stencil3_wgrad: bad channel counts");
  SV_REQUIRE((((uintptr_t)x | (uintptr_t)dy) & (act_dtype == SV_BF16 ? 7 : 15)) == 0, "stencil3_wgrad: operands must be aligned to 4 elements");
  SV_REQUIRE(groups == 1 || groups == 3, "stencil3_wgrad: unsupported groups=%d", groups);
    const int ntiles = I * (D / (groups == 3 ? StencilBrick<3>::TZV : StencilBrick<1>::TZV)) * (H / TY) * (W / TX);
  hipStream_t s = (hipStream_t)stream;
  SV_DISPATCH_ACT(act_dtype,
    const int per_cu = groups == 1 ? resident_per_cu((const void*)stencil3_wgrad_kernel<1, AT>, StencilBrick<1>::NTHR)
                                   : resident_per_cu((const void*)stencil3_wgrad_kernel<3, AT>, StencilBrick<3>::NTHR);
    const int resident = 256 * per_cu;
    const int blocks = ntiles < resident ? ntiles : resident;
    StencilWArgsT<AT> a{static_cast<const AT*>(x), ldx, cin_load, x_plane_stride, static_cast<const AT*>(dy), lddy, cout_load, dw, workspace, dbias, cout, cin, c_stride, c_valid,
                        I, D, H, W, ntiles};
    if (groups == 1) hipLaunchKernelGGL((stencil3_wgrad_kernel<1, AT>), dim3(blocks), dim3(StencilBrick<1>::NTHR), 0, s, a);
    else hipLaunchKernelGGL((stencil3_wgrad_kernel<3, AT>), dim3(blocks), dim3(StencilBrick<3>::NTHR), 0, s, a););
  if (workspace) hipLaunchKernelGGL(stencil_wgrad_fold_kernel, dim3(cdiv(cout * cin * 27, 256)), dim3(256), 0, s, workspace, dw, cout * cin * 27);
  return check_launch("sv_stencil3_wgrad");
}

extern "C" int sv_tconv4s2_fwd(const void* x, const void* w_packed, const float* bias, void* out, double* stats, int I, int D, int H, int W,
                               int cin, int cout, void* stream) {
  SV_REQUIRE(x && w_packed && out && I > 0, "tconv4s2_fwd: null argument");
  SV_REQUIRE(cin == 32 && cout > 0 && cout <= 8, "tconv4s2_fwd: built for 32 input and <= 8 output channels (got %d -> %d)", cin, cout);
  SV_REQUIRE(D % T4_JZ == 0 && H % T4_JY == 0 && W % T4_JX == 0, "tconv4s2_fwd: input grid %dx%dx%d must be a multiple of the 4x4x8 brick", D, H, W);
  SV_REQUIRE((((uintptr_t)x | (uintptr_t)w_packed | (uintptr_t)out) & 15) == 0, "tconv4s2_fwd: operands must be 16-byte aligned");
  TConv4Args a{static_cast<const __bf16*>(x), static_cast<const __bf16*>(w_packed), bias, static_cast<__bf16*>(out), stats, cout, I, D, H, W,
               I * (D / T4_JZ) * (H / T4_JY) * (W / T4_JX)};
  const int blocks = a.nbricks < 512 ? a.nbricks : 512;
  hipLaunchKernelGGL(tconv4s2_fwd_kernel, dim3(blocks), dim3(256), 0, (hipStream_t)stream, a);
  return check_launch("sv_tconv4s2_fwd");
}
```

### swinvox_amd/hip.py

```python
from __future__ import annotations

import ctypes as C
import os
import threading

import torch

_HERE = os.path.dirname(os.path.abspath(__file__))
LIB_PATH = os.environ.get("SV_HIP_LIB") or os.path.join(_HERE, "libswinvox_hip.so")

ACT_NONE, ACT_RELU, ACT_GELU, ACT_LRELU = 0, 1, 2, 3
MATH_F32, MATH_BF16, MATH_FP8, MATH_FP8_FULL = 0, 1, 2, 3
F32, BF16 = 0, 1


class Geom(C.Structure):
    _fields_ = [(n, C.c_int) for n in ("N", "Di", "Hi", "Wi", "Do", "Ho", "Wo", "Ci", "Co", "kd", "kh", "kw",
                                        "sd", "sh", "sw", "pd", "ph", "pw", "ldi")]


class Epilogue(C.Structure):
    _fields_ = [("bias", C.c_void_p), ("residual", C.c_void_p), ("ldr", C.c_int), ("row_scale", C.c_void_p),
                ("rows_per_scale", C.c_int), ("pre_act", C.c_void_p), ("stats", C.c_void_p), ("act", C.c_int),
                ("slope", C.c_float), ("act_grad_src", C.c_void_p), ("act_grad_kind", C.c_int), ("ldc", C.c_int),
                ("col_off", C.c_int)]


class PackDesc(C.Structure):
    _fields_ = [("src", C.c_void_p), ("dst", C.c_void_p), ("A", C.c_int), ("B", C.c_int), ("T", C.c_int), ("swap", C.c_int),
                ("rows_out", C.c_int), ("inner_out", C.c_int), ("block0", C.c_int), ("reserved", C.c_int)]


class AugSample(C.Structure):
    _fields_ = [("bg", C.c_float * 3), ("jitter_value", C.c_float * 3), ("jitter_order", C.c_int * 3), ("noise", C.c_float * 3),
                ("perm", C.c_int * 3), ("mean", C.c_float * 3), ("std", C.c_float * 3)]


_P, _I, _L, _F, _U, _D = C.c_void_p, C.c_int, C.c_longlong, C.c_float, C.c_uint32, C.c_double
_ACT_TYPED = {
    "sv_conv_gather", "sv_tconv_gather", "sv_conv_wgrad", "sv_stencil3_fwd", "sv_stencil3_wgrad", "sv_colsum",
    "sv_layernorm_fwd", "sv_layernorm_bwd", "sv_ln_image_fwd", "sv_ln_image_bwd", "sv_bn_stats", "sv_scale_shift_act", "sv_bn_bwd", "sv_scale_shift_act_signs", "sv_bn_bwd_signs",
    "sv_window_attention_fwd", "sv_window_attention_bwd", "sv_cross_view_attention_fwd", "sv_cross_view_attention_bwd",
    "sv_transpose", "sv_add_n", "sv_axpby", "sv_relu_bwd", "sv_maxpool2d_fwd", "sv_maxpool2d_bwd", "sv_avgpool2_fwd", "sv_avgpool2_bwd",
    "sv_decoder_seed_fwd", "sv_decoder_seed_bwd", "sv_maxpool3d_fwd", "sv_maxpool3d_bwd", "sv_dropout", "sv_rowscale",
    "sv_dwconv2x2_fwd", "sv_dwconv2x2_bwd", "sv_upsample3to7_add_fwd", "sv_upsample3to7_bwd",
    "sv_cva_downsample_fwd", "sv_cva_downsample_bwd", "sv_cva_upsample_add_fwd", "sv_cva_upsample_bwd", "sv_decoder_head_fwd", "sv_decoder_head_bwd",
    "sv_merge_views_fwd", "sv_merge_views_bwd", "sv_stem_space_to_depth", "sv_encoder_prep", "sv_encoder_prep_bwd", "sv_bn_act_maxpool_fwd", "sv_bn_maxpool_bwd", "sv_bn_act_maxpool3d_fwd", "sv_bn_maxpool3d_bwd", "sv_head_pack_x", "sv_head_unpack_dx", "sv_swin_attn_block_fwd", "sv_swin_attn_block_bwd",
    "sv_linear_fp8", "sv_linear_fp8_dgrad",
}
_PROTOS = {
    "sv_version": (_I, None),
    "sv_conv_gather": (_I, [_P, _P, _P, C.POINTER(Geom), C.POINTER(Epilogue), _I]),
    "sv_tconv_gather": (_I, [_P, _P, _P, C.POINTER(Geom), C.POINTER(Epilogue), _I]),
    "sv_conv_gather_is_wide": (_I, None, [_P, _P, _P, C.POINTER(Geom), C.POINTER(Epilogue), _I, _I]),
    "sv_conv_wgrad_is_wide": (_I, None, [_P, _I, _P, C.POINTER(Geom), _I, _I, _I]),
    "sv_conv_wgrad_workspace_floats": (C.c_size_t, None, [C.POINTER(Geom)]),
    "sv_conv_wgrad": (_I, [_P, _I, _P, _P, C.POINTER(Geom), _I, _P, _P, _I]),
    "sv_quant_rows_e4m3": (_I, [_P, _I, _I, _I, _I, _P, _I, _P]),
    "sv_linear_fp8": (_I, [_P, _P, _P, _P, _P, _I, _I, _I, C.POINTER(Epilogue)]),
    "sv_linear_fp8_supported": (_I, None, [_I, _I, C.POINTER(Epilogue), _I, _I]),
    "sv_linear_fp8_launches": (_L, None),
    "sv_quant_cols_e4m3": (_I, [_P, _I, _I, _I, _I, _P, _I, _P, _P]),
    "sv_linear_fp8_dgrad": (_I, [_P, _P, _P, _P, _P, _I, _I, _I, C.POINTER(Epilogue)]),
    "sv_linear_fp8_dgrad_supported": (_I, None, [_I, _I, C.POINTER(Epilogue), _I, _I]),
    "sv_linear_fp8_wgrad": (_I, [_P, _P, _P, _P, _P, _I, _I, _I, _I, _I]),
    "sv_linear_fp8_bwd_launches": (_L, None, [_I]),
    "sv_stencil3_fwd": (_I, [_P, _I, _I, _I, _P, _I, _P, _P, _I, _I, _I, _P, _I, _P, _I, _I, _I, _I, _L, _L]),
    "sv_stencil3_wgrad_workspace_floats": (C.c_size_t, None, [_I, _I]),
    "sv_stencil3_wgrad": (_I, [_P, _I, _I, _I, _P, _I, _I, _P, _P, _P, _I, _I, _I, _I, _I, _I, _I, _I, _L]),
    "sv_tconv4s2_fwd": (_I, [_P, _P, _P, _P, _P, _I, _I, _I, _I, _I, _I]),
    "sv_pack_weight": (_I, [_P, _P, _I, _I, _I, _I, _I, _I]),
    "sv_pack_weights_block_elems": (_I, None),
    "sv_pack_weights": (_I, [_P, _I, _I, _I]),
    "sv_colsum": (_I, [_P, _I, _I, _I, _P, _I]),
    "sv_cast": (_I, [_P, _I, _P, _I, _L]),
    "sv_layernorm_fwd": (_I, [_P, _P, _P, _P, _P, _P, _L, _I, _F, _I, _I]),
    "sv_layernorm_bwd_workspace_floats": (C.c_size_t, None, [_I]),
    "sv_layernorm_bwd": (_I, [_P, _P, _P, _P, _P, _P, _P, _P, _P, _L, _I, _I, _I, _I]),
    "sv_bn_bwd_workspace_doubles": (C.c_size_t, None, [_I]),
    "sv_ln_image_workspace_floats": (C.c_size_t, None, [_I, _I]),
    "sv_ln_image_fwd": (_I, [_P, _P, _P, _P, _P, _P, _I, _I, _F, _F, _U, _P]),
    "sv_ln_image_bwd": (_I, [_P, _P, _P, _P, _P, _P, _P, _P, _I, _I, _F, _U, _P]),
    "sv_bn_stats": (_I, [_P, _L, _I, _I, _P]),
    "sv_bn_finalize": (_I, [_P, _L, _P, _P, _P, _P, _F, _F, _I, _P, _P, _P, _P, _I]),
    "sv_scale_shift_act": (_I, [_P, _I, _P, _P, _P, _I, _P, _I, _L, _I, _I, _F]),
    "sv_bn_bwd": (_I, [_P, _I, _P, _I, _P, _I, _P, _P, _P, _L, _I, _I, _F, _I, _P, _I, _P, _I, _P, _P, _P, _P, _P]),
    "sv_bn_signs_supported": (_I, None, [_I]),
    "sv_scale_shift_act_signs": (_I, [_P, _I, _P, _P, _P, _I, _P, _I, _L, _I, _I, _F, _P]),
    "sv_bn_bwd_signs": (_I, [_P, _I, _P, _P, _I, _P, _P, _P, _L, _I, _I, _F, _I, _P, _I, _P, _I, _P, _P, _P]),
    "sv_window_attention_fwd": (_I, [_P, _P, _P, _I, _I, _I, _I, _I, _I, _I]),
    "sv_window_attention_bwd_workspace_floats": (C.c_size_t, None, [_I]),
    "sv_window_attention_windows_per_group": (_I, None, [_I, _I, _I, _I, _I, _I]),
    "sv_window_attention_bwd": (_I, [_P, _P, _P, _P, _P, _P, _I, _I, _I, _I, _I, _I, _I]),
    "sv_stem_space_to_depth": (_I, [_P, _P, _I]),
    "sv_bn_act_maxpool_fwd": (_I, [_P, _P, _P, _P, _P, _I, _I, _I, _I, _I, _F]),
    "sv_bn_maxpool_bwd": (_I, [_P, _P, _P, _P, _P, _P, _P, _P, _I, _I, _I, _I, _I, _F, _I, _P, _P, _P, _P]),
    "sv_bn_act_maxpool3d_fwd": (_I, [_P, _P, _P, _P, _P, _I, _I, _I, _I, _I, _I, _F]),
    "sv_bn_maxpool3d_bwd": (_I, [_P, _P, _P, _P, _P, _P, _P, _P, _I, _I, _I, _I, _I, _I, _F, _I, _P, _P, _P, _P]),
    "sv_set_conv_halo": (_I, None, [_I]),
    "sv_conv_halo_mode": (_I, None),
    "sv_set_conv_halo_wgrad": (_I, None, [_I]),
    "sv_conv_halo_launches": (_L, None),
    "sv_encoder_prep": (_I, [_P, _I, _P, _P, _I, _I]),
    "sv_encoder_prep_bwd": (_I, [_P, _P, _P, _I, _I, _I]),
    "sv_head_pack_x": (_I, [_P, _P, _I, _I]),
    "sv_head_unpack_dx": (_I, [_P, _P, _I, _I]),
    "sv_stem_pack": (_I, [_P, _P, _I]),
    "sv_stem_unpack_grad": (_I, [_P, _P]),
    "sv_stem_native": (_I, [_P, _P]),
    "sv_merger_pack": (_I, [_P, _P, _I, _I, _I, _I]),
    "sv_swin_mlp_supported": (_I, None, [_I]),
    "sv_swin_mlp_pack": (_I, [_P, _P, _P, _I]),
    "sv_swin_mlp_fwd": (_I, [_P, _P, _P, _P, _P, _P, _P, _P, _I, _L, _I, _F]),
    "sv_swin_mlp_bwd": (_I, [_P, _P, _P, _P, _P, _P, _P, _P, _I, _P, _P, _L, _I, _F]),
    "sv_swin_mlp_wgrad": (_I, [_P, _P, _P, _P, _P, _P, _P, _P, _I, _P, _P, _P, _P, _L, _I, _F]),
    "sv_swin_attn_block_supported": (_I, None, [_I, _I, _I, _I]),
    "sv_swin_attn_block_windows_per_group": (_I, None, [_I, _I, _I, _I]),
    "sv_swin_attn_block_fwd": (_I, [_P] * 15 + [_I, _I, _I, _I, _I, _I, _F]),
    "sv_swin_attn_block_bwd": (_I, [_P] * 17 + [_I, _I, _I, _I, _I, _I]),
    "sv_cross_view_attention_fwd": (_I, [_P, _P, _I, _I, _I, _I, _I]),
    "sv_cross_view_attention_bwd": (_I, [_P, _P, _P, _I, _I, _I, _I, _I]),
    "sv_transpose": (_I, [_P, _P, _I, _I, _I, _I, _I, _L, _L]),
    "sv_add_n": (_I, [_P, _P, _P, _P, _P, _L, _I, _I]),
    "sv_axpby": (_I, [_P, _P, _P, _F, _F, _L]),
    "sv_relu_bwd": (_I, [_P, _P, _P, _L]),
    "sv_maxpool2d_fwd": (_I, [_P, _P, _P, _I, _I, _I, _I]),
    "sv_maxpool2d_bwd": (_I, [_P, _P, _P, _I, _I, _I, _I]),
    "sv_avgpool2_fwd": (_I, [_P, _P, _I, _I, _I, _I, _I, _I]),
    "sv_avgpool2_bwd": (_I, [_P, _P, _I, _I, _I, _I, _I, _I]),
    "sv_decoder_seed_fwd": (_I, [_P, _P, _I, _I]),
    "sv_decoder_seed_bwd": (_I, [_P, _P, _I, _I]),
    "sv_maxpool3d_fwd": (_I, [_P, _P, _P, _I, _I, _I, _I, _I]),
    "sv_maxpool3d_bwd": (_I, [_P, _P, _P, _I, _I, _I, _I, _I]),
    "sv_dropout": (_I, [_P, _P, _L, _F, _U, _P]),
    "sv_droppath_scale": (_I, [_P, _I, _F, _U, _P]),
    "sv_rowscale": (_I, [_P, _P, _P, _L, _I, _I]),
    "sv_dwconv2x2_fwd": (_I, [_P, _P, _P, _P, _I, _I]),
    "sv_dwconv2x2_bwd": (_I, [_P, _P, _P, _P, _P, _P, _I, _I]),
    "sv_upsample3to7_add_fwd": (_I, [_P, _P, _I, _P, _I, _I]),
    "sv_upsample3to7_bwd": (_I, [_P, _P, _I, _I]),
    "sv_cva_downsample_fwd": (_I, [_P, _P, _P, _P, _I, _I, _I]),
    "sv_cva_downsample_bwd": (_I, [_P, _P, _P, _P, _P, _P, _I, _I, _I]),
    "sv_cva_upsample_add_fwd": (_I, [_P, _P, _I, _P, _I, _I, _I]),
    "sv_cva_upsample_bwd": (_I, [_P, _P, _I, _I, _I]),
    "sv_decoder_head_fwd": (_I, [_P, _P, _P, _P, _P, _L]),
    "sv_decoder_head_bwd": (_I, [_P, _P, _P, _P, _P, _P, _P, _L]),
    "sv_merge_views_fwd": (_I, [_P, _P, _P, _I, _I, _I]),
    "sv_merge_views_bwd": (_I, [_P, _P, _P, _P, _P, _P, _I, _I, _I]),
    "sv_mean_views": (_I, [_P, _P, _I, _I, _I]),
    "sv_bce_logits": (_I, [_P, _P, _L, _P, _P, _P]),
    "sv_iou_counts": (_I, [_P, _P, _P, _I, _I, _I, _P]),
    "sv_binvox_decode": (_I, [_P, _P, _I, _I, _I, _I, _I, _P, _P]),
    "sv_augment_views": (_I, [_P, _I, _I, _I, _I, _I, _I, _I, _I, _I, _P, _P, _P, _P]),
    "sv_grad_sumsq": (_I, [_P, _L, _F, _P]),
    "sv_adam_step": (_I, [_P, _P, _P, _P, _L, _D, _D, _D, _D, _D, _L, _F, _P, _F, _P]),
    "sv_sgd_step": (_I, [_P, _P, _P, _L, _D, _D, _D, _L, _F, _P, _F, _P]),
}


def _argtypes(name):
    spec = _PROTOS[name]
    if spec[1] is None:
        return list(spec[2]) if len(spec) > 2 else []
    return list(spec[1]) + ([_I] if name in _ACT_TYPED else []) + [_P]


def kernel_source_hash() -> str:
    import glob
    import hashlib
    h = hashlib.sha256()
    files = sorted(glob.glob(os.path.join(_HERE, "csrc", "*.hip")) + glob.glob(os.path.join(_HERE, "csrc", "*.h")))
# ... 127 lines not shown
```

### swinvox_amd/models/_base.py

```python
from __future__ import annotations

from typing import Dict, List, Sequence

import torch
import torch.nn as nn

from .. import hip, ops
from ..ops import ACT_LRELU, ACT_NONE, ACT_RELU, BatchNormState, ConvSpec, call, empty, ptr, zeros


class GradStore:

    def __init__(self, params: Sequence[torch.Tensor], layout=None):
        from ..optim import FlatLayout
        self.params = list(params)
        self._map: Dict[int, torch.Tensor] = {}
        self.flat = None
        if self.params:
            layout = layout if layout is not None else FlatLayout(self.params)
            self.flat = torch.zeros(layout.total, dtype=torch.float32, device=self.params[0].device)
            for p, v in zip(self.params, layout.views(self.flat)):
                self._map[id(p)] = v

    def __getitem__(self, p: torch.Tensor) -> torch.Tensor:
# ... 37 lines not shown
        arena = mod.__dict__.setdefault("_arena_b", ops.ZeroArena())
        ops.set_arena(arena)
        aw = ops.AsyncWgrad(grads.flat.device) if ops.overlap_enabled() else None
        ops.set_async_wgrad(aw)
        try:
            arena.begin(douts[0].device if douts[0] is not None else grads.flat.device)
            d_inputs = mod._bwd(ctx.tape, grads, ctx.in_needs, *douts)
        finally:
            ops.set_async_wgrad(None)
            if aw is not None:
                aw.join()
            arena.end()
            ops.set_pack_cache(None)
            ops.set_arena(None)
        ctx.tape = None
        return (None, None, None) + tuple(d_inputs) + grads.as_tuple()


class HipModule(nn.Module):

    stochastic = True
    grad_ready_hook = None

    def _announce(self, grads: "GradStore", group_index: int) -> None:
        hook = self.grad_ready_hook
        if hook is None:
            return
        views = [grads[p] for p in self._grad_groups_cached()[group_index] if p.requires_grad]
        if not views:
            return
        if not views[0].is_cuda:
            hook(group_index, views)
            return
        cur = torch.cuda.current_stream()
        cs = ops.comm_stream(views[0].device)
        cs.wait_stream(cur)
        aw = ops._CTX.awg
        if aw is not None:
            cs.wait_stream(aw.stream)
        with torch.cuda.stream(cs):
            hook(group_index, views)

    def _grad_groups_cached(self):
        pl = self._param_list()
        gg = self.__dict__.get("_ggroups")
        if gg is None or gg[0] != len(pl):
            gg = self.__dict__["_ggroups"] = (len(pl), self.grad_groups())
        return gg[1]

    def _param_list(self) -> List[torch.Tensor]:
        pl = self.__dict__.get("_plist")
        if pl is None or len(pl) != self.__dict__.get("_plist_n", -1):
            pl = list(self.parameters())
            self.__dict__["_plist"], self.__dict__["_plist_n"] = pl, len(pl)
        return pl

    def _grad_layout(self):
        from ..optim import FlatLayout
        pl = self._param_list()
        lay = self.__dict__.get("_glayout")
        if lay is None or not lay.matches(pl):
            lay = self.__dict__["_glayout"] = FlatLayout(pl)
        return lay

    def _run(self, *inputs):
        hip.check_cuda(*inputs)
        hip.check_cuda(*self._param_list()[:1])
        for t in inputs:
            if t.dtype != torch.float32 and t.dtype != ops._STATE["store"]:
                raise RuntimeError(f"swinvox_amd: expected float32 inputs, got {t.dtype}")
        params = self._param_list()
        save = torch.is_grad_enabled() and (any(p.requires_grad for p in params) or any(t.requires_grad for t in inputs))
        return _ModuleFn.apply(self, len(inputs), save, *inputs, *params)

    def _seed(self) -> int:
        return int(torch.randint(0, 2 ** 31 - 1, (1,)).item())


class ConvBnAct:

    def __init__(self, conv: nn.Module, bn: nn.Module, spec: ConvSpec, act: int, slope: float = 0.0):
        self.conv, self.bn, self.spec, self.act, self.slope = conv, bn, spec, act, slope

    def forward(self, x, n, in_grid, training, *, ldi=None, z=None, ldz=None, residual=None, ldr=0):
        sp = self.spec
        og = sp.out_grid(in_grid)
        M = n * og[0] * og[1] * og[2]
        wf = self._pack("f")
        y = empty(M, sp.cout, like=x)
        st = BatchNormState(self.bn, M, training)
        sp.forward(x, n, in_grid, wf, y, ldi=ldi, bias=self.conv.bias, stats=st.sums)
        st.finalize()
        if z is None:
            z, ldz = empty(M, sp.cout, like=x), sp.cout
        st.apply(y, sp.cout, z, ldz, self.act, self.slope, residual, ldr)
        return z, og, (x, ldi, y, z if residual is not None else None, ldz, st, n, in_grid, M)

    def backward(self, ctx, dz, lddz, grads, *, need_dx=True, dres=None, lddres=0, dx=None, lddx=None, dx_epi=None):
        x, ldi, y, z, ldz, st, n, in_grid, M = ctx
        sp = self.spec
        dy = (zeros if sp.cout_mem != sp.cout else empty)(M, sp.cout_mem, like=dz)
        st.backward(dz, lddz, z, ldz, y, sp.cout, dy, sp.cout_mem, grads[self.bn.weight], grads[self.bn.bias], self.act, self.slope,
                    dres, lddres)
        sp.wgrad(dy, x, n, in_grid, self._dw(grads), lddy=sp.cout_mem, ldx=ldi,
                 db=grads[self.conv.bias] if self.conv.bias is not None else None)
        if not need_dx:
            return None
        Min = n * in_grid[0] * in_grid[1] * in_grid[2]
        if dx is None:
            dx = (zeros if sp.cin_mem != sp.cin else empty)(Min, sp.cin_mem, like=dz)
            lddx = sp.cin_mem
        sp.dgrad(dy, n, in_grid, self._pack("d"), dx, lddy=sp.cout_mem, lddx=lddx, **(dx_epi or {}))
        return dx

    def forward_pool3d(self, x, n, in_grid, training):
        sp = self.spec
        og = sp.out_grid(in_grid)
        M = n * og[0] * og[1] * og[2]
        y = empty(M, sp.cout, like=x)
        st = BatchNormState(self.bn, M, training)
        sp.forward(x, n, in_grid, self._pack("f"), y, bias=self.conv.bias, stats=st.sums)
        st.finalize()
        st.probe(y, sp.cout)
        pg = (og[0] // 2, og[1] // 2, og[2] // 2)
        p = empty(n * pg[0] * pg[1] * pg[2], sp.cout, like=x)
        idx = torch.empty(p.numel(), dtype=torch.uint8, device=x.device)
        call("sv_bn_act_maxpool3d_fwd", ptr(y), ptr(st.scale), ptr(st.shift), ptr(p), ptr(idx), n, og[0], og[1], og[2], sp.cout, self.act, self.slope)
        return p, og, (x, y, st, n, in_grid, og, M, idx)

    def backward_pool3d(self, ctx, dp, grads, *, need_dx=True):
        x, y, st, n, in_grid, og, M, idx = ctx
        sp = self.spec
        assert sp.cout_mem == sp.cout
        dy = empty(M, sp.cout, like=dp)
        ws = ops.zeros_f64((ops.BN_BWD_SLOTS + 1) * 2 * sp.cout + 2, dp.device)
        call("sv_bn_maxpool3d_bwd", ptr(dp), ptr(idx), ptr(y), ptr(self.bn.weight), ptr(st.mean), ptr(st.rstd), ptr(st.scale), ptr(st.shift),
             n, og[0], og[1], og[2], sp.cout, self.act, self.slope, 1 if st.training else 0, ptr(dy), ptr(grads[self.bn.weight]), ptr(grads[self.bn.bias]),
             ptr(ws))
        sp.wgrad(dy, x, n, in_grid, self._dw(grads), lddy=sp.cout, db=grads[self.conv.bias] if self.conv.bias is not None else None)
        if not need_dx:
            return None
        Min = n * in_grid[0] * in_grid[1] * in_grid[2]
        dx = (zeros if sp.cin_mem != sp.cin else empty)(Min, sp.cin_mem, like=dp)
        sp.dgrad(dy, n, in_grid, self._pack("d"), dx, lddy=sp.cout, lddx=sp.cin_mem)
        return dx

    def _pack(self, kind):
        return self.spec.pack_fwd(self.conv.weight) if kind == "f" else self.spec.pack_dgrad(self.conv.weight)

    def _dw(self, grads):
        return grads[self.conv.weight]


def conv_spec_of(m: nn.Module, **kw) -> ConvSpec:
    if isinstance(m, nn.Linear):
        return ConvSpec.linear(m.in_features, m.out_features)
    if isinstance(m, nn.Conv2d):
        assert m.groups == 1 and m.dilation == (1, 1)
        return ConvSpec.conv2d(m.in_channels, m.out_channels, m.kernel_size, m.stride, m.padding, **kw)
    if isinstance(m, nn.ConvTranspose3d):
        assert m.groups == 1 and m.output_padding == (0, 0, 0)
        return ConvSpec.conv3d(m.in_channels, m.out_channels, m.kernel_size, m.stride, m.padding, transposed=True, **kw)
    if isinstance(m, nn.Conv3d):
        assert m.groups == 1
        return ConvSpec.conv3d(m.in_channels, m.out_channels, m.kernel_size, m.stride, m.padding, **kw)
    raise TypeError(type(m))
```

### swinvox_amd/models/encoder.py

```python
from __future__ import annotations

import logging
from typing import List

import torch
import torch.nn as nn

from .. import ops
from ..ops import ACT_NONE, ACT_RELU, BatchNormState, ConvSpec, call, empty, ptr, zeros
from ._base import ConvBnAct, HipModule, conv_spec_of
from .cross_view_attention import CrossViewAttention
from .swin_transformer import SwinTransformer, swin_backward, swin_forward


class Bottleneck(nn.Module):
    def __init__(self, inplanes, planes, stride, with_downsample):
        super().__init__()
        self.conv1 = nn.Conv2d(inplanes, planes, 1, bias=False)
        self.bn1 = nn.BatchNorm2d(planes)
        self.conv2 = nn.Conv2d(planes, planes, 3, stride=stride, padding=1, bias=False)
        self.bn2 = nn.BatchNorm2d(planes)
        self.conv3 = nn.Conv2d(planes, planes * 4, 1, bias=False)
        self.bn3 = nn.BatchNorm2d(planes * 4)
        self.relu = nn.ReLU(inplace=True)
        self.downsample = None
        if with_downsample:
            self.downsample = nn.Sequential(nn.Conv2d(inplanes, planes * 4, 1, stride=stride, bias=False), nn.BatchNorm2d(planes * 4))
        self.stride = stride
        self._c1 = ConvBnAct(self.conv1, self.bn1, conv_spec_of(self.conv1), ACT_RELU)
        self._c2 = ConvBnAct(self.conv2, self.bn2, conv_spec_of(self.conv2), ACT_RELU)
        self._c3 = ConvBnAct(self.conv3, self.bn3, conv_spec_of(self.conv3), ACT_RELU)
        self._cd = ConvBnAct(self.downsample[0], self.downsample[1], conv_spec_of(self.downsample[0]), ACT_NONE) if with_downsample else None

    def fwd(self, x, n, grid, training):
        a, g1, c1 = self._c1.forward(x, n, grid, training)
        b, g2, c2 = self._c2.forward(a, n, g1, training)
        idt, cd = x, None
        if self._cd is not None:
            idt, _, cd = self._cd.forward(x, n, grid, training)
        out, g3, c3 = self._c3.forward(b, n, g2, training, residual=idt, ldr=self.conv3.out_channels)
        return out, g3, (c1, c2, c3, cd)

    def bwd(self, ctx, dout, grads):
        c1, c2, c3, cd = ctx
        Co = self.conv3.out_channels
        didt = empty(dout.shape[0], Co, like=dout)
        db = self._c3.backward(c3, dout, Co, grads, dres=didt, lddres=Co)
        da = self._c2.backward(c2, db, self.conv2.out_channels, grads)
        skip = self._cd.backward(cd, didt, Co, grads) if cd is not None else didt
        return self._c1.backward(c1, da, self.conv1.out_channels, grads, dx_epi=dict(residual=skip, ldr=self.conv1.in_channels))


def _res_layer(inplanes, planes, blocks, stride):
    return nn.Sequential(Bottleneck(inplanes, planes, stride, True), *[Bottleneck(planes * 4, planes, 1, False) for _ in range(blocks - 1)])


class Encoder(HipModule):
    def __init__(self, cfg, variant: str = "tiny"):
        super().__init__()
        self.cfg = cfg
        n = cfg.NETWORK
        logging.info("swinvox_amd: ResNet-50 / Swin weights are randomly initialised (no network); load a checkpoint to restore them")
        self.resnet = nn.Sequential(
            nn.Conv2d(3, 64, 7, stride=2, padding=3, bias=False), nn.BatchNorm2d(64), nn.ReLU(inplace=True),
            nn.MaxPool2d(3, stride=2, padding=1), _res_layer(64, 64, 3, 1), _res_layer(256, 128, 4, 2), _res_layer(512, 256, 6, 2))
        self.swin_transformer = SwinTransformer(cfg, in_channels=3, img_size=224, pretrained=True, variant=variant)
        self.resnet_reduce = nn.Conv2d(1024, 256, kernel_size=1)
        if n.USE_SWIN_T_MULTI_STAGE:
            self.swin_stage_reduces = nn.ModuleList([nn.Conv2d(ch, 256, kernel_size=1) for ch in self.swin_transformer.out_channels])
            chains = []
            for i in n.SWIN_T_STAGES:
                nblk = 3 - i if i <= 2 else 0
                mods = []
                for _ in range(nblk):
                    mods += [nn.Conv2d(256, 256, kernel_size=3, stride=2, padding=1), nn.BatchNorm2d(256), nn.ReLU()]
                chains.append(nn.Sequential(*mods) if nblk else nn.Identity())
            self.swin_downsamples = nn.ModuleList(chains)
        else:
            self.swin_reduce = nn.Conv2d(self.swin_transformer.out_channels[-1], 256, kernel_size=1)
        self.cross_view_attention = CrossViewAttention(cfg, in_channels=512) if n.USE_CROSS_VIEW_ATTENTION else None

        def cbr(cin):
            return nn.Sequential(nn.Conv2d(cin, 256, kernel_size=3, padding=1), nn.BatchNorm2d(256), nn.ReLU())

        self.fusion_layer, self.layer1, self.layer2, self.layer3 = cbr(512), cbr(256), cbr(256), cbr(256)
        self._stem_spec = ConvSpec.conv2d(16, 64, 4, 1, 2, og_fixed=(1, 112, 112))
        self._s_rr = ConvSpec.linear(1024, 256)
        self._post = [ConvBnAct(m[0], m[1], conv_spec_of(m[0]), ACT_RELU) for m in (self.fusion_layer, self.layer1, self.layer2, self.layer3)]
        if n.USE_SWIN_T_MULTI_STAGE:
            self._s_red = [ConvSpec.linear(c.in_channels, 256) for c in self.swin_stage_reduces]
            self._chains = [[ConvBnAct(ch[3 * j], ch[3 * j + 1], conv_spec_of(ch[3 * j]), ACT_RELU) for j in range(len(ch) // 3)]
                            if not isinstance(ch, nn.Identity) else [] for ch in self.swin_downsamples]
        else:
            self._s_red1 = ConvSpec.linear(self.swin_reduce.in_channels, 256)

    def grad_groups(self):
        res = list(self.resnet.parameters())
        swin = list(self.swin_transformer.parameters())
        skip = {id(p) for p in res} | {id(p) for p in swin}
        tail = [p for p in self.parameters() if id(p) not in skip]
        return [tail, swin, res]

    def forward(self, rendering_images):
        assert rendering_images.dim() == 5 and rendering_images.shape[2] == 3, "expected [B, V, 3, H, W]"
        assert tuple(rendering_images.shape[-2:]) == (224, 224), "swinvox_amd: images must be 224x224 (reference cfg.CONST.IMG_H/W)"
        if self.cross_view_attention is not None and rendering_images.shape[1] > 32:
            raise RuntimeError("swinvox_amd: cross-view attention keeps all views of a sample in LDS: n_views must be <= 32 "
                               f"(got {rendering_images.shape[1]}; the reference's data sets render 24)")
        return self._run(rendering_images)

    def _stem_pack(self):
        wp = empty(64 * 16 * 16, like=self.resnet[0].weight)
        call("sv_stem_pack", ptr(self.resnet[0].weight), ptr(wp), ops.hip.ACT)
        return wp

    def _stem_fwd(self, images, I, tr, x16=None):
        if x16 is None:
            x16 = empty(I * 112 * 112, 16, like=images)
            call("sv_stem_space_to_depth", ptr(images), ptr(x16), I)
        sp, bn, M = self._stem_spec, self.resnet[1], I * 112 * 112
        y = empty(M, 64, like=x16)
        st = BatchNormState(bn, M, tr)
        sp.forward(x16, I, (1, 112, 112), self._stem_pack(), y, stats=st.sums)
# ... 190 lines not shown
```

### swinvox_amd/models/merger.py

```python
from __future__ import annotations

import torch
import torch.nn as nn

from .. import ops
from ..ops import ACT_LRELU, BatchNormState, ConvSpec, call, empty, fzeros, ptr, zeros
from ._base import HipModule
from .decoder import VOX, as_channels_last12, raw_view

G = (32, 32, 32)


class Merger(HipModule):
    def __init__(self, cfg):
        super().__init__()
        self.cfg = cfg
        lk = cfg.NETWORK.LEAKY_VALUE
        self._slope = float(lk)

        def c3(cin, cout):
            return nn.Sequential(nn.Conv3d(cin, cout, kernel_size=3, padding=1), nn.BatchNorm3d(cout), nn.LeakyReLU(lk))

        self.layer1, self.layer2, self.layer3, self.layer4 = c3(9, 9), c3(9, 9), c3(9, 9), c3(9, 9)
        self.layer5 = c3(36, 9)
        self.layer6 = c3(9, 1)
        self._s14 = ConvSpec.conv3d(9, 9, 3, 1, 1, cin_mem=12, cout_mem=12)
        self._s5 = ConvSpec.conv3d(48, 9, 3, 1, 1, cin_mem=48, cout_mem=12)
        self._s6 = ConvSpec.conv3d(9, 1, 3, 1, 1, cin_mem=12, cout_mem=4)
        idx = torch.tensor([12 * g + j for g in range(4) for j in range(9)], dtype=torch.long)
        self.register_buffer("_cat_cols", idx, persistent=False)

    def forward(self, raw_features, coarse_volumes):
        assert raw_features.dim() == 6 and tuple(raw_features.shape[2:]) == (9, 32, 32, 32), "raw_features must be [B,V,9,32,32,32]"
        assert tuple(coarse_volumes.shape) == (raw_features.shape[0], raw_features.shape[1], 32, 32, 32)
        return self._run(raw_features, coarse_volumes)

    def _layer(self, li):
        return (self.layer1, self.layer2, self.layer3, self.layer4, self.layer5, self.layer6)[li]

    def _spec(self, li):
        return self._s14 if li < 4 else (self._s5 if li == 4 else self._s6)

    def _w5_padded(self):
        w5 = self.layer5[0].weight
        wp = fzeros(9, 48, 27, like=w5)
        wp[:, self._cat_cols] = w5.detach().reshape(9, 36, 27)
        return wp

    def _stencil_pack(self, li, dgrad):
        w = self._layer(li)[0].weight
        wp = torch.empty(16 * 27 * (48 if li == 4 else 16), dtype=torch.bfloat16, device=w.device)
        call("sv_merger_pack", ptr(w), ptr(wp), w.shape[0], w.shape[1], 1 if dgrad else 0, 1 if li == 4 else 0)
        return wp

    def _conv_fwd(self, li, x, ldi, y, ldc, stats, w5p=None):
        conv, I = self._layer(li)[0], y.shape[0] // VOX
        if ops.get_math() == "bf16":
            call("sv_stencil3_fwd", ptr(x), ldi, 48 if li == 4 else 12, 3 if li == 4 else 1, ptr(self._stencil_pack(li, False)), 1,
                 ptr(conv.bias), ptr(y), ldc, 0, conv.out_channels, None, 0, ptr(stats), I, 32, 32, 32, I * VOX * 12 if li == 4 else 0, 0)
        else:
            sp = self._spec(li)
            sp.forward(x, I, G, sp.pack_fwd(w5p if li == 4 else conv.weight), y, ldi=ldi, ldc=ldc, bias=conv.bias, stats=stats)

    def _conv_dgrad(self, li, dy, lddy, dx, lddx, accumulate, w5p=None):
        conv, I = self._layer(li)[0], dy.shape[0] // VOX
        if ops.get_math() == "bf16":
            call("sv_stencil3_fwd", ptr(dy), lddy, lddy if lddy <= 12 else 12, 1, ptr(self._stencil_pack(li, True)), 3 if li == 4 else 1,
                 None, ptr(dx), lddx, 0, 48 if li == 4 else 9, ptr(dx) if accumulate else None, lddx, None, I, 32, 32, 32,
                 0, I * VOX * 12 if li == 4 else 0)
        else:
            sp = self._spec(li)
            epi = dict(residual=dx, ldr=lddx) if accumulate else {}
            sp.dgrad(dy, I, G, sp.pack_dgrad(w5p if li == 4 else conv.weight), dx, lddy=lddy, lddx=lddx, **epi)

    def _conv_wgrad(self, li, dy, lddy, x, ldx, grads):
        conv, I = self._layer(li)[0], dy.shape[0] // VOX
        if ops.get_math() == "bf16":
            ws = ops.zeros_f64(8 * conv.out_channels * conv.in_channels * 27, dy.device)
            call("sv_stencil3_wgrad", ptr(x), ldx, 48 if li == 4 else 12, 3 if li == 4 else 1, ptr(dy), lddy, lddy if lddy <= 12 else 12,
                 ptr(grads[conv.weight]), ptr(grads[conv.bias]), ptr(ws), conv.out_channels, conv.in_channels, 12 if li == 4 else 16, 9, I, 32, 32, 32,
                 I * VOX * 12 if li == 4 else 0)
        elif li == 4:
            dw5p = fzeros(9, 48, 27, like=dy)
            self._s5.wgrad(dy, x, I, G, dw5p, lddy=lddy, ldx=ldx, async_ok=False)
            grads[conv.weight].view(9, 36, 27).copy_(dw5p[:, self._cat_cols])
        else:
            self._spec(li).wgrad(dy, x, I, G, grads[conv.weight], lddy=lddy, ldx=ldx)

    def _bias_grad(self, dy, M, C, ld, db):
        if ops.get_math() != "bf16":
            ops.colsum(dy, M, C, ld, db)

    def _fwd(self, raw, vol, save):
        B, V = raw.shape[:2]
        M, tr, sl = B * V * VOX, self.training, self._slope
        raw_dtype, vol_dtype = raw.dtype, vol.dtype
        x12 = ops.to_store(as_channels_last12(raw))
        vol = ops.to_store(vol)
        planar = ops.get_math() == "bf16"
        buf = empty if planar else zeros
        cat = empty(4, M, 12, like=vol) if planar else zeros(M, 48, like=vol)
        ldz = 12 if planar else 48
        w5p = self._w5_padded() if not planar else None
        ctx14, xin, ldi = [], x12, 12
        for k in range(4):
            bn = self._layer(k)[1]
            y = empty(M, 12, like=vol)
            st = BatchNormState(bn, M, tr)
            self._conv_fwd(k, xin, ldi, y, 12, st.sums)
            st.finalize()
            z = cat[k] if planar else cat[:, 12 * k:]
            st.apply(y, 12, z, ldz, ACT_LRELU, sl)
            ctx14.append((xin, ldi, y, z, st))
            xin, ldi = z, ldz
        y5 = empty(M, 12, like=vol)
        st5 = BatchNormState(self.layer5[1], M, tr)
        self._conv_fwd(4, cat, ldz, y5, 12, st5.sums, w5p)
        st5.finalize()
        z5 = buf(M, 12, like=vol)
        st5.apply(y5, 12, z5, 12, ACT_LRELU, sl)
        y6 = empty(M, 1, like=vol)
        st6 = BatchNormState(self.layer6[1], M, tr)
        self._conv_fwd(5, z5, 12, y6, 1, st6.sums)
        st6.finalize()
        wl = empty(M, 1, like=vol)
        st6.apply(y6, 1, wl, 1, ACT_LRELU, sl)
        out = empty(B, 32, 32, 32, like=vol)
        call("sv_merge_views_fwd", ptr(wl), ptr(vol), ptr(out), B, V, VOX)
        tape = (B, V, x12, vol, cat, ctx14, w5p, y5, st5, z5, y6, st6, wl, out, raw_dtype, vol_dtype) if save else None
        return ops.to_f32(out), tape

    def _bwd(self, tape, grads, in_needs, dout):
        B, V, x12, vol, cat, ctx14, w5p, y5, st5, z5, y6, st6, wl, out, raw_dtype, vol_dtype = tape
        M, sl = B * V * VOX, self._slope
        dout = ops.to_store(dout)
        dwl = empty(M, 1, like=vol)
        dvol = empty(B, V, 32, 32, 32, like=vol)
        call("sv_merge_views_bwd", ptr(wl), ptr(vol), ptr(out), ptr(dout), ptr(dwl), ptr(dvol), B, V, VOX)
        conv6, bn6 = self.layer6[0], self.layer6[1]
        dy6 = zeros(M, 4, like=vol)
        st6.backward(dwl, 1, None, 0, y6, 1, dy6, 4, grads[bn6.weight], grads[bn6.bias], ACT_LRELU, sl)
        self._bias_grad(dy6, M, 1, 4, grads[conv6.bias])
        self._conv_wgrad(5, dy6, 4, z5, 12, grads)
        buf = empty if ops.get_math() == "bf16" else zeros
        dz5 = buf(M, 12, like=vol)
        self._conv_dgrad(5, dy6, 4, dz5, 12, False)
        conv5, bn5 = self.layer5[0], self.layer5[1]
        dy5 = buf(M, 12, like=vol)
        st5.backward(dz5, 12, None, 0, y5, 12, dy5, 12, grads[bn5.weight], grads[bn5.bias], ACT_LRELU, sl)
        self._bias_grad(dy5, M, 9, 12, grads[conv5.bias])
        planar = cat.dim() == 3
        ldz = 12 if planar else 48
        self._conv_wgrad(4, dy5, 12, cat, ldz, grads)
        dcat = empty(4, M, 12, like=vol) if planar else zeros(M, 48, like=vol)
        self._conv_dgrad(4, dy5, 12, dcat, ldz, False, w5p)
        dx = None
        for k in (3, 2, 1, 0):
            conv, bn = self._layer(k)[0], self._layer(k)[1]
            xin, ldi, y, z, st = ctx14[k]
            dzk = dcat[k] if planar else dcat[:, 12 * k:]
            dy = buf(M, 12, like=vol)
            st.backward(dzk, ldz, None, 0, y, 12, dy, 12, grads[bn.weight], grads[bn.bias], ACT_LRELU, sl)
            self._bias_grad(dy, M, 9, 12, grads[conv.bias])
            self._conv_wgrad(k, dy, 12, xin, ldi, grads)
            if k > 0:
                self._conv_dgrad(k, dy, 12, dcat[k - 1] if planar else dcat[:, 12 * (k - 1):], ldz, True)
            else:
                dx = buf(M, 12, like=vol)
                self._conv_dgrad(k, dy, 12, dx, 12, False)
        draw = raw_view(dx if raw_dtype == dx.dtype else ops.to_f32(dx), B, V) if in_needs[0] else None
        return (draw, (dvol if vol_dtype == dvol.dtype else ops.to_f32(dvol)) if in_needs[1] else None)
```

### swinvox_amd/ops.py

```python
from __future__ import annotations

import ctypes as C
import threading
from dataclasses import dataclass
from typing import Optional, Tuple

import torch

from . import hip
from .hip import ACT_GELU, ACT_LRELU, ACT_NONE, ACT_RELU, Epilogue, Geom, call, ptr

_STATE = {"math": hip.MATH_F32, "store": torch.float32}


class _CallContext(threading.local):
    packs = None
    arena = None
    awg = None
    bn_tick = None


_CTX = _CallContext()
BN_SLOTS = 16
BN_BWD_SLOTS, LN_BWD_SLOTS = 16, 32
# ... 493 lines not shown
            return
    linear_fwd(x, rows, spec, w, out, **epi)


def quantize_cols_fp8(t: torch.Tensor, rows: int, Cc: int, ld: Optional[int] = None, colsum: Optional[torch.Tensor] = None):
    Mp = (rows + 127) // 128 * 128
    q = torch.empty(Cc, Mp, dtype=torch.uint8, device=t.device)
    sc = torch.empty(Cc, dtype=torch.float32, device=t.device)
    call("sv_quant_cols_e4m3", ptr(t), hip.BF16 if t.dtype == torch.bfloat16 else hip.F32, rows, Cc, ld or Cc, ptr(q), Mp, ptr(sc), ptr(colsum))
    return q, sc


def quantize_weight_t_fp8(w: torch.Tensor):
    cache = _CTX.packs
    if cache is None or not isinstance(w, torch.nn.Parameter):
        return quantize_cols_fp8(w, w.shape[0], w.shape[1])
    hit = cache.w8t.get(id(w))
    if hit is None:
        hit = cache.w8t[id(w)] = quantize_cols_fp8(w, w.shape[0], w.shape[1])
    return hit


def _fp8_bwd_site(spec: ConvSpec, w) -> bool:
    return (linear_fp8_bwd_enabled() and spec.taps == 1 and spec.cin_mem == spec.cin and spec.cout_mem == spec.cout
            and isinstance(w, torch.nn.Parameter))


def swin_linear_dgrad(dy, rows, spec: ConvSpec, w, dx, **epi):
    if _fp8_bwd_site(spec, w):
        e = _epilogue(spec.cin, **epi)
        if hip.load().sv_linear_fp8_dgrad_supported(spec.cout, spec.cin, C.byref(e), _STATE["math"], hip.ACT) == 1:
            dq, sd = quantize_rows_fp8(dy, rows, spec.cout)
            wtq, swt = quantize_weight_t_fp8(w)
            traced_call("sv_linear_fp8_dgrad", 2.0 * rows * spec.cin * spec.cout, float(rows) * (dq.shape[1] + dy.element_size() * spec.cin) + wtq.numel(),
                        ptr(dq), ptr(sd), ptr(wtq), ptr(swt), ptr(dx), rows, spec.cout, spec.cin, C.byref(e), tag=f"M={rows} N={spec.cout} K={spec.cin}")
            return
    linear_dgrad(dy, rows, spec, spec.pack_dgrad(w), dx, **epi)


def swin_linear_wgrad(dy, x, rows, spec: ConvSpec, w, dw, db=None, async_ok=True):
    if not _fp8_bwd_site(spec, w):
        return linear_wgrad(dy, x, rows, spec, dw, db, async_ok=async_ok)

    def run():
        dyt, sdc = quantize_cols_fp8(dy, rows, spec.cout, colsum=db)
        xt, sxc = quantize_cols_fp8(x, rows, spec.cin)
        traced_call("sv_linear_fp8_wgrad", 2.0 * rows * spec.cin * spec.cout, float(dyt.numel() + xt.numel()) + 8.0 * spec.cin * spec.cout,
                    ptr(dyt), ptr(sdc), ptr(xt), ptr(sxc), ptr(dw), rows, spec.cout, spec.cin, spec.cin, 0, tag=f"M={rows} N={spec.cout} K={spec.cin}")

    aw = _CTX.awg
    if aw is not None and async_ok:
        aw.stream.wait_stream(torch.cuda.current_stream())
        aw.held.append((dy, x))
        with torch.cuda.stream(aw.stream):
            run()
        return
    run()


def linear_dgrad(dy, rows, spec: ConvSpec, w_t, dx, **epi):
    spec.dgrad(dy, rows, (1, 1, 1), w_t, dx, **epi)


def linear_wgrad(dy, x, rows, spec: ConvSpec, dw, db=None, async_ok=True):
    spec.wgrad(dy, x, rows, (1, 1, 1), dw, db=db, async_ok=async_ok)


def layernorm_fwd(x, gamma, beta, rows, Cdim, merge_hw=(0, 0), eps=1e-5):
    y = empty(rows, Cdim, like=x)
    mean = fempty(rows, like=x)
    rstd = fempty(rows, like=x)
    call("sv_layernorm_fwd", ptr(x), ptr(gamma), ptr(beta), ptr(y), ptr(mean), ptr(rstd), rows, Cdim, eps, merge_hw[0], merge_hw[1])
    return y, mean, rstd


def layernorm_bwd(dy, x, gamma, mean, rstd, dx, dgamma, dbeta, rows, Cdim, merge_hw=(0, 0), accumulate_dx=False):
    ws = zeros_f64(LN_BWD_SLOTS * Cdim + 1, dy.device)
    call("sv_layernorm_bwd", ptr(dy), ptr(x), ptr(gamma), ptr(mean), ptr(rstd), ptr(dx), ptr(dgamma), ptr(dbeta), ptr(ws), rows, Cdim,
         merge_hw[0], merge_hw[1], 1 if accumulate_dx else 0)


class BatchNormState:

    def __init__(self, bn: torch.nn.Module, M: int, training: bool):
        self.bn, self.M, self.training, self.C = bn, M, training, bn.num_features
        dev = bn.weight.device
        self.sums = zeros_f64(BN_SLOTS * 2 * self.C, dev) if training else None
        buf = fempty(4 * self.C, device=dev)
        self.scale, self.shift, self.mean, self.rstd = buf[:self.C], buf[self.C:2 * self.C], buf[2 * self.C:3 * self.C], buf[3 * self.C:]

    def finalize(self):
        bn = self.bn
        if self.training and bn.num_batches_tracked is not None:
            if _CTX.bn_tick is None:
                _CTX.bn_tick = []
            _CTX.bn_tick.append(bn.num_batches_tracked)
        mom = bn.momentum if bn.momentum is not None else 0.1
        call("sv_bn_finalize", ptr(self.sums), self.M, ptr(bn.weight), ptr(bn.bias), ptr(bn.running_mean), ptr(bn.running_var),
             float(mom), float(bn.eps), 1 if self.training else 0, ptr(self.scale), ptr(self.shift), ptr(self.mean), ptr(self.rstd), self.C)

    def probe(self, x, ldx):
        probe = _STATE.get("bn_probe")
        if probe is not None:
            probe(self, x, ldx)

    def apply(self, x, ldx, y, ldy, act=ACT_NONE, slope=0.0, residual=None, ldr=0):
        self.probe(x, ldx)
        self.signs = None
        if (residual is not None and act != ACT_NONE and self.training and _bn_signs_on() and self.C % 256 == 0
                and self.C % 4 == 0 and ldx % 4 == 0 and ldy % 4 == 0 and ldr % 4 == 0):
            self.signs = torch.empty(self.M * (self.C // 64), dtype=torch.int64, device=x.device)
            call("sv_scale_shift_act_signs", ptr(x), ldx, ptr(self.scale), ptr(self.shift), ptr(residual), ldr, ptr(y), ldy, self.M, self.C, act, slope,
                 ptr(self.signs))
            return
        call("sv_scale_shift_act", ptr(x), ldx, ptr(self.scale), ptr(self.shift), ptr(residual), ldr, ptr(y), ldy, self.M, self.C, act, slope)

    def backward(self, dz, lddz, z, ldz, x, ldx, dx, lddx, dgamma, dbeta, act=ACT_NONE, slope=0.0, dres=None, lddres=0):
        ws = zeros_f64((BN_BWD_SLOTS + 1) * 2 * self.C + 2, dz.device)
        if getattr(self, "signs", None) is not None and dres is not None:
            call("sv_bn_bwd_signs", ptr(dz), lddz, ptr(self.signs), ptr(x), ldx, ptr(self.bn.weight), ptr(self.mean), ptr(self.rstd), self.M, self.C,
                 act, slope, 1 if self.training else 0, ptr(dx), lddx, ptr(dres), lddres, ptr(dgamma), ptr(dbeta), ptr(ws))
            return
        call("sv_bn_bwd", ptr(dz), lddz, ptr(z), ldz, ptr(x), ldx, ptr(self.bn.weight), ptr(self.mean), ptr(self.rstd), self.M, self.C,
             act, slope, 1 if self.training else 0, ptr(dx), lddx, ptr(dres), lddres, ptr(dgamma), ptr(dbeta), ptr(ws),
             ptr(self.scale), ptr(self.shift))


def _bn_signs_on() -> bool:
    import os
    return _STATE.get("bn_signs", os.environ.get("SV_BN_SIGNS", "1") != "0")


def set_bn_signs(on: bool) -> None:
    _STATE["bn_signs"] = bool(on)


def input_prep_enabled() -> bool:
    import os
    return _STATE.get("input_prep", os.environ.get("SV_INPUT_PREP", "1") != "0")


def set_input_prep(on: bool) -> None:
    _STATE["input_prep"] = bool(on)


def bn_pool_fused_enabled() -> bool:
    import os
    return _STATE.get("bn_pool_fused", os.environ.get("SV_BN_POOL_FUSED", "1") != "0")


def set_bn_pool_fused(on: bool) -> None:
    _STATE["bn_pool_fused"] = bool(on)


def set_conv_halo(mode: int) -> None:
    rc = hip.load().sv_set_conv_halo(int(mode))
    if rc != 0:
        raise RuntimeError(f"sv_set_conv_halo failed (rc={rc}): {hip.load().sv_last_error().decode()}")


def set_conv_halo_wgrad(mode: int) -> None:
    rc = hip.load().sv_set_conv_halo_wgrad(int(mode))
    if rc != 0:
        raise RuntimeError(f"sv_set_conv_halo_wgrad failed (rc={rc}): {hip.load().sv_last_error().decode()}")


def set_bn_probe(fn) -> None:
    _STATE["bn_probe"] = fn


def transpose(src, dst, batch, R, Cc, lds=None, ldd=None, sb=None, db=None):
    lds = lds or Cc
    ldd = ldd or R
    assert src.dtype == dst.dtype
    call("sv_transpose", ptr(src), ptr(dst), batch, R, Cc, lds, ldd, sb if sb is not None else R * lds, db if db is not None else Cc * ldd,
         act=hip.BF16 if src.dtype == torch.bfloat16 else hip.F32)
```

Baseline: 4804 views/s.

## Fold BN+LeakyReLU into stencil conv halo loads and residual scale-shift pass

Adds BN-folded variants of the 3D stencil forward and wgrad kernels. They apply the previous layer's scale/shift and LeakyReLU while loading the input halo, so the merger no longer materialises the normalized activations with a separate scale_shift_act pass. It also adds a signs-path scale-shift kernel that normalizes the residual in the same pass, for a fold_skip option. The wgrad path recomputes the activation, and the new forward variant uses a higher occupancy bound. Together these add per-element ALU work and register pressure inside the stencil kernels.

```diff
diff --git a/include/swinvox_hip.h b/include/swinvox_hip.h
--- a/include/swinvox_hip.h
+++ b/include/swinvox_hip.h
@@ -80,6 +80,13 @@
 int sv_stencil3_wgrad(const void* x, int ldx, int cin_load, int groups, const void* dy, int lddy, int cout_load,
                       float* dw, float* dbias, float* workspace, int cout, int cin, int c_stride, int c_valid, int I, int D, int H, int W,
                       long long x_plane_stride, int act_dtype, void* stream);
+int sv_stencil3_fwd_bn(const void* x, int ldx, int cin_load, int groups, const void* w_bf16, int ntiles16, const float* bias, void* out, int ldc,
+                       int col_off, int cout, const void* residual, int ldr, double* stats, int I, int D, int H, int W,
+                       long long x_plane_stride, long long out_plane_stride, const float* bn_tab, int tab_ld, int act, float slope,
+                       int act_dtype, void* stream);
+int sv_stencil3_wgrad_bn(const void* x, int ldx, int cin_load, int groups, const void* dy, int lddy, int cout_load, float* dw, float* dbias,
+                         float* workspace, int cout, int cin, int c_stride, int c_valid, int I, int D, int H, int W, long long x_plane_stride,
+                         const float* bn_tab, int tab_ld, int act, float slope, int act_dtype, void* stream);
 int sv_tconv4s2_fwd(const void* x, const void* w_packed, const float* bias, void* out, double* stats, int I, int D, int H, int W,
                     int cin, int cout, void* stream);
 int sv_pack_weight(const float* src, void* dst, int A, int B, int T, int swap, int pad_to, int out_dtype, void* stream);
@@ -129,6 +136,9 @@
 int sv_bn_signs_supported(int C);
 int sv_scale_shift_act_signs(const void* x, int ldx, const float* scale, const float* shift, const void* residual, int ldr, void* y, int ldy,
                              long long M, int C, int act, float slope, void* signs, int act_dtype, void* stream);
+int sv_scale_shift_act_signs_res(const void* x, int ldx, const float* scale, const float* shift, const void* residual, int ldr,
+                                 const float* res_scale, const float* res_shift, void* y, int ldy, long long M, int C, int act, float slope,
+                                 void* signs, int act_dtype, void* stream);
 int sv_bn_bwd_signs(const void* dz, int lddz, const void* signs, const void* x, int ldx, const float* gamma, const float* save_mean,
                     const float* save_rstd, long long M, int C, int act, float slope, int training, void* dx, int lddx, void* dres, int lddres,
                     float* dgamma, float* dbeta, double* sums_ws, int act_dtype, void* stream);
diff --git a/swinvox_amd/csrc/common.h b/swinvox_amd/csrc/common.h
--- a/swinvox_amd/csrc/common.h
+++ b/swinvox_amd/csrc/common.h
@@ -200,6 +200,10 @@
     default: return v;
   }
 }
+__device__ __forceinline__ float bn_affine(float x, float scale, float shift) { return __fmaf_rn(x, scale, shift); }
+__device__ __forceinline__ float bn_act(float x, float scale, float shift, int act, float slope) {
+  return apply_act(bn_affine(x, scale, shift), act, slope);
+}
 __device__ __forceinline__ float act_grad(float pre, int act, float slope) {
   switch (act) {
     case SV_ACT_RELU: return pre > 0.f ? 1.f : 0.f;
diff --git a/swinvox_amd/csrc/norm.hip b/swinvox_amd/csrc/norm.hip
--- a/swinvox_amd/csrc/norm.hip
+++ b/swinvox_amd/csrc/norm.hip
@@ -635,23 +635,30 @@
   }
 }
 
-template <typename AT>
+template <typename AT, bool RESBN = false>
 __global__ __launch_bounds__(256) void scale_shift_act_cg_kernel(const AT* __restrict__ x, int ldx, const float* __restrict__ scale,
                                                                  const float* __restrict__ shift, const AT* __restrict__ res, int ldr,
                                                                  AT* __restrict__ y, int ldy, long long M, int C, int act, float slope,
-                                                                 long long rows_per_block, int G, unsigned long long* __restrict__ signs) {
+                                                                 long long rows_per_block, int G, unsigned long long* __restrict__ signs,
+                                                                 const float* __restrict__ res_scale, const float* __restrict__ res_shift) {
   const int gq = threadIdx.x % G, rl = threadIdx.x / G, RL = 256 / G;
   const int c = (blockIdx.x * G + gq) * 4;
   if (c >= C || rl >= RL) return;
   const float4 sc = *reinterpret_cast<const float4*>(scale + c), sh = *reinterpret_cast<const float4*>(shift + c);
+  float4 rsc = make_float4(0.f, 0.f, 0.f, 0.f), rsh = rsc;
+  if constexpr (RESBN) { rsc = *reinterpret_cast<const float4*>(res_scale + c); rsh = *reinterpret_cast<const float4*>(res_shift + c); }
   const long long r0 = (long long)blockIdx.y * rows_per_block;
   long long r1 = r0 + rows_per_block; if (r1 > M) r1 = M;
 #pragma unroll 2
   for (long long r = r0 + rl; r < r1; r += RL) {
     const float4 xv = ld4f(x + (size_t)r * ldx + c);
-    float o[4] = {__fmaf_rn(xv.x, sc.x, sh.x), __fmaf_rn(xv.y, sc.y, sh.y), __fmaf_rn(xv.z, sc.z, sh.z), __fmaf_rn(xv.w, sc.w, sh.w)};
+    float o[4] = {bn_affine(xv.x, sc.x, sh.x), bn_affine(xv.y, sc.y, sh.y), bn_affine(xv.z, sc.z, sh.z), bn_affine(xv.w, sc.w, sh.w)};
     if (res) {
-      const float4 rv = ld4f(res + (size_t)r * ldr + c);
+      float4 rv = ld4f(res + (size_t)r * ldr + c);
+      if constexpr (RESBN) {
+        rv.x = (float)(AT)bn_affine(rv.x, rsc.x, rsh.x); rv.y = (float)(AT)bn_affine(rv.y, rsc.y, rsh.y);
+        rv.z = (float)(AT)bn_affine(rv.z, rsc.z, rsh.z); rv.w = (float)(AT)bn_affine(rv.w, rsc.w, rsh.w);
+      }
       o[0] += rv.x; o[1] += rv.y; o[2] += rv.z; o[3] += rv.w;
     }
     if (signs) {
@@ -1231,7 +1238,8 @@
 static inline bool bn_signs_ok(int C) { return C % 256 == 0; }
 
 static int scale_shift_act_impl(const void* x, int ldx, const float* scale, const float* shift, const void* residual, int ldr,
-                                void* y, int ldy, long long M, int C, int act, float slope, unsigned long long* signs, int act_dtype, void* stream) {
+                                void* y, int ldy, long long M, int C, int act, float slope, unsigned long long* signs, int act_dtype, void* stream,
+                                const float* res_scale = nullptr, const float* res_shift = nullptr) {
   SV_REQUIRE(x && scale && shift && y && M > 0 && C > 0 && ldx >= C && ldy >= C, "scale_shift_act: bad arguments");
   SV_REQUIRE_ACT(act_dtype);
   hipStream_t s = (hipStream_t)stream;
@@ -1240,6 +1248,8 @@
   const bool narrow = !vec && C <= BN_NARROW_MAXC && (ldx % 4 == 0) && (ldy % 4 == 0) && ldx >= ((C + 3) & ~3) && ldy >= ((C + 3) & ~3) &&
                       (!residual || (ldr % 4 == 0 && ldr >= ((C + 3) & ~3))) && aligned4(act_dtype, x, y, residual);
   SV_REQUIRE(!signs || (vec && bn_signs_ok(C) && ((uintptr_t)signs & 15) == 0), "scale_shift_act_signs: needs C %% 256 == 0 and 4-aligned rows (C=%d)", C);
+  SV_REQUIRE(!res_scale || (signs && residual && res_shift && (((uintptr_t)res_scale | (uintptr_t)res_shift) & 15) == 0),
+             "scale_shift_act_signs_res: the residual's scale / shift need the sign-word path, a residual and 16-byte alignment");
   if (narrow) {
     long long blocks = (M + 63) / 64; if (blocks > 8192) blocks = 8192;
     SV_DISPATCH_ACT(act_dtype, hipLaunchKernelGGL(scale_shift_act_narrow_kernel<AT>, dim3((unsigned)blocks), dim3(256), 0, s, static_cast<const AT*>(x), ldx, scale, shift,
@@ -1250,8 +1260,12 @@
     long long splits = 4096 / cg; if (splits < 1) splits = 1;
     const long long maxs = (M + 4 * RL - 1) / (4 * RL); if (splits > maxs) splits = maxs;
     const long long rpb = (M + splits - 1) / splits;
-    SV_DISPATCH_ACT(act_dtype, hipLaunchKernelGGL(scale_shift_act_cg_kernel<AT>, dim3(cg, cdiv(M, rpb)), dim3(256), 0, s, static_cast<const AT*>(x), ldx, scale, shift,
-                                                  static_cast<const AT*>(residual), ldr, static_cast<AT*>(y), ldy, M, C, act, slope, rpb, G, signs););
+    if (res_scale)
+      SV_DISPATCH_ACT(act_dtype, hipLaunchKernelGGL((scale_shift_act_cg_kernel<AT, true>), dim3(cg, cdiv(M, rpb)), dim3(256), 0, s, static_cast<const AT*>(x), ldx, scale, shift,
+                                                    static_cast<const AT*>(residual), ldr, static_cast<AT*>(y), ldy, M, C, act, slope, rpb, G, signs, res_scale, res_shift););
+    else
+      SV_DISPATCH_ACT(act_dtype, hipLaunchKernelGGL((scale_shift_act_cg_kernel<AT, false>), dim3(cg, cdiv(M, rpb)), dim3(256), 0, s, static_cast<const AT*>(x), ldx, scale, shift,
+                                                    static_cast<const AT*>(residual), ldr, static_cast<AT*>(y), ldy, M, C, act, slope, rpb, G, signs, nullptr, nullptr););
   } else {
     long long blocks = (M * C + 255) / 256; if (blocks > 8192) blocks = 8192;
     SV_DISPATCH_ACT(act_dtype, hipLaunchKernelGGL(scale_shift_act_scalar_kernel<AT>, dim3((unsigned)blocks), dim3(256), 0, s, static_cast<const AT*>(x), ldx, scale, shift,
@@ -1269,6 +1283,14 @@
                                         void* y, int ldy, long long M, int C, int act, float slope, void* signs, int act_dtype, void* stream) {
   SV_REQUIRE(signs, "scale_shift_act_signs: null sign buffer");
   return scale_shift_act_impl(x, ldx, scale, shift, residual, ldr, y, ldy, M, C, act, slope, static_cast<unsigned long long*>(signs), act_dtype, stream);
+}
+
+extern "C" int sv_scale_shift_act_signs_res(const void* x, int ldx, const float* scale, const float* shift, const void* residual, int ldr,
+                                            const float* res_scale, const float* res_shift, void* y, int ldy, long long M, int C, int act,
+                                            float slope, void* signs, int act_dtype, void* stream) {
+  SV_REQUIRE(signs && residual && res_scale && res_shift, "scale_shift_act_signs_res: null argument");
+  return scale_shift_act_impl(x, ldx, scale, shift, residual, ldr, y, ldy, M, C, act, slope, static_cast<unsigned long long*>(signs), act_dtype, stream,
+                              res_scale, res_shift);
 }
 
 static bool bn_pool_shape_ok(int N, int H, int W, int C) {
diff --git a/swinvox_amd/csrc/stencil.hip b/swinvox_amd/csrc/stencil.hip
--- a/swinvox_amd/csrc/stencil.hip
+++ b/swinvox_amd/csrc/stencil.hip
@@ -17,6 +17,8 @@
   return b;
 }
 __device__ __forceinline__ bf16x4 to_bf16x4(bf16x4 v) { return v; }
+__device__ __forceinline__ float r4(const float4& v, int j) { return j == 0 ? v.x : j == 1 ? v.y : j == 2 ? v.z : v.w; }
+__device__ __forceinline__ float r4(const bf16x4& v, int j) { return (float)v[j]; }
 
 __device__ __forceinline__ int xcd_first_tile() {
   const int n = gridDim.x, b = blockIdx.x;
@@ -32,10 +34,17 @@
   return r;
 }
 
-template <int G, typename AT, int TZV = TZ, int NTHR = 256>
+constexpr int halo_gcd(int a, int b) { return b == 0 ? a : halo_gcd(b, a % b); }
+struct HaloBn { const float* tab; int tab_ld; int act; float slope; };
+template <int G, typename AT, int TZV = TZ, int NTHR = 256, bool BN = false>
 struct HaloRegs {
   static constexpr int HZV = TZV + 2, HPOSV = HZV * HY * HX;
   static constexpr int C = 16 * G, VPP = C / 4, N = (HPOSV * VPP + NTHR - 1) / NTHR;
+  static constexpr int NPH = BN ? VPP / halo_gcd(VPP, NTHR) : 1;
+  int tcv[NPH];
+  const float* tl;
+  int out_, act_;
+  float slope_;
   typedef typename std::conditional<G == 1, int, long long>::type OffT;
   typename V4<AT>::type r[N];
   OffT off[N];
@@ -54,6 +63,21 @@
       lds[k] = ((hz * HY + hy) * pitch + hx) * C + cv;
     }
   }
+  __device__ __forceinline__ void init_bn(const HaloBn& bn, float* tlw, int ldx, long long plane, int cin_load, int tid) {
+    act_ = bn.act; slope_ = bn.slope; out_ = 0; tl = tlw;
+    if (tid < VPP) {
+      const int cv = tid * 4, pl = plane ? cv / ldx : 0;
+      float4 sc = make_float4(0.f, 0.f, 0.f, 0.f), sh = sc;
+      if (cv < cin_load) {
+        const float* row = bn.tab + (size_t)pl * 2 * bn.tab_ld + (cv - pl * ldx);
+        sc = *reinterpret_cast<const float4*>(row); sh = *reinterpret_cast<const float4*>(row + bn.tab_ld);
+      }
+      *reinterpret_cast<float4*>(tlw + cv) = sc; *reinterpret_cast<float4*>(tlw + C + cv) = sh;
+    }
+#pragma unroll
+    for (int ph = 0; ph < NPH; ++ph) tcv[ph] = ((tid + NTHR * ph) % VPP) * 4;
+    __syncthreads();
+  }
   __device__ __forceinline__ void load(const AT* __restrict__ x, int ldx, const TileId& t, int D, int H, int W) {
     const int out = (t.z0 == 0 ? 1 : 0) | (t.z0 + TZV == D ? 2 : 0) | (t.y0 == 0 ? 4 : 0) | (t.y0 + TY == H ? 8 : 0) | (t.x0 == 0 ? 16 : 0) | (t.x0 + TX == W ? 32 : 0) | 64;
     const AT* corner = x + ((((long long)t.img * D + t.z0 - 1) * H + t.y0 - 1) * W + t.x0 - 1) * (long long)ldx;
@@ -65,12 +89,25 @@
 #endif
       r[k] = q;
     }
+    if constexpr (BN) out_ = out;
   }
   __device__ __forceinline__ void store(__bf16* Xs, int tid) const {
+    if constexpr (BN) __builtin_assume(act_ != SV_ACT_GELU);
 #pragma unroll
     for (int k = 0; k < N; ++k) {
       const int i = tid + NTHR * k;
-      if (i < HPOSV * VPP) *reinterpret_cast<bf16x4*>(Xs + lds[k]) = to_bf16x4(r[k]);
+      if (i < HPOSV * VPP) {
+        bf16x4 b = to_bf16x4(r[k]);
+        if constexpr (BN) {
+          if ((face[k] & out_) == 0) {
+            const float4 sc = *reinterpret_cast<const float4*>(tl + tcv[k % NPH]), sh = *reinterpret_cast<const float4*>(tl + C + tcv[k % NPH]);
+            b = to_bf16x4(make_float4(bn_act((float)r4(r[k], 0), sc.x, sh.x, act_, slope_), bn_act((float)r4(r[k], 1), sc.y, sh.y, act_, slope_),
+                                      bn_act((float)r4(r[k], 2), sc.z, sh.z, act_, slope_), bn_act((float)r4(r[k], 3), sc.w, sh.w, act_, slope_)));
+          }
+        }
+        *reinterpret_cast<bf16x4*>(Xs + lds[k]) = b;
+      }
+      if constexpr (BN) __builtin_amdgcn_sched_barrier(0);
     }
   }
 };
@@ -84,18 +121,20 @@
   const AT* residual; int ldr;
   double* stats;
   int I, D, H, W, ntiles;
+  HaloBn bn;
 };
 
 template <int G> struct StencilPitch { static constexpr int HXP = G == 1 ? 16 : HX; };
 template <int G> struct StencilBrick { static constexpr int TZV = 8, NTHR = TZV * 64; };
 template <int G> struct StencilBrickF { static constexpr int TZV = 8, NTHR = TZV * 64; };
-template <int G, int NT, typename AT, bool VEC>
-__global__ __launch_bounds__(StencilBrickF<G>::NTHR, 2) void stencil3_fwd_kernel(const StencilArgsT<AT> p) {
+template <int G, int NT, typename AT, bool VEC, bool BN = false>
+__global__ __launch_bounds__(StencilBrickF<G>::NTHR, (BN && G == 1 && NT == 1) ? 4 : 2) void stencil3_fwd_kernel(const StencilArgsT<AT> p) {
   constexpr int C = 16 * G, KTOT = 27 * C, KPAD = (KTOT + 31) / 32 * 32, NSTEP = KPAD / 32, HXP = StencilPitch<G>::HXP;
   constexpr int TZV = StencilBrickF<G>::TZV, NTHR = StencilBrickF<G>::NTHR, NW = NTHR / 64;
   __shared__ __attribute__((aligned(16))) char xc[(TZV + 2) * HY * HXP * C * 2];
   __shared__ __attribute__((aligned(16))) __bf16 Ws[NT * 16 * KPAD];
   __shared__ float red[16 * 16 * 2];
+  __shared__ __attribute__((aligned(16))) float bntab[BN ? 2 * C : 4];
   __bf16* Xs = reinterpret_cast<__bf16*>(xc);
   const int tid = threadIdx.x, lane = tid & 63, wave = tid >> 6;
   const int lr = lane & 15, lg = lane >> 4;
@@ -113,8 +152,9 @@
 #pragma unroll
     for (int j = 0; j < 4; ++j) { const int n = nt * 16 + lg * 4 + j; bias4[nt][j] = (p.bias && n < p.cout) ? p.bias[n] : 0.f; }
 
-  HaloRegs<G, AT, TZV, NTHR> hr;
+  HaloRegs<G, AT, TZV, NTHR, BN> hr;
   hr.init(p.ldx, p.x_plane, p.cin_load, p.H, p.W, tid, HXP);
+  if constexpr (BN) hr.init_bn(p.bn, bntab, p.ldx, p.x_plane, p.cin_load, tid);
   int tile = xcd_first_tile();
   TileId t = tile_of<TZV>(tile < p.ntiles ? tile : 0, p.D, p.H, p.W);
   if (tile < p.ntiles) { hr.load(p.x, p.ldx, t, p.D, p.H, p.W); hr.store(Xs, tid); }
@@ -179,7 +219,7 @@
           for (int j = 0; j < 4; ++j) v[j] = colreal[nt][j] ? acc[mt][nt][j] + bias4[nt][j] : 0.f;
           if (NT == 1 && p.stats) {
 #pragma unroll
-            for (int j = 0; j < 4; ++j) { st1[j] += v[j]; st2[j] += v[j] * v[j]; }
+            for (int j = 0; j < 4; ++j) { st1[j] += v[j]; st2[j] = __fmaf_rn(v[j], v[j], st2[j]); }
           }
           if (p.residual) {
             const float4 rv = ld4f(rrow + (size_t)mt * 2 * p.W * p.ldr);
@@ -202,7 +242,7 @@
           for (int j = 0; j < 4; ++j) {
             if (nn + j < p.cout) {
               float r = acc[mt][nt][j] + bias4[nt][j];
-              if (NT == 1 && p.stats) { st1[j] += r; st2[j] += r * r; }
+              if (NT == 1 && p.stats) { st1[j] += r; st2[j] = __fmaf_rn(r, r, st2[j]); }
               if (p.residual) r += ldf(p.residual + pos * p.ldr + nn + j);
               stf(p.out + pos * p.ldc + p.col_off + nn + j, r);
             }
@@ -248,6 +288,7 @@
   int cout, cin;
   int c_stride, c_valid;
   int I, D, H, W, ntiles;
+  HaloBn bn;
 };
 
 constexpr int WG_SLOTS = 16;
@@ -260,13 +301,14 @@
   dw[i] += a;
 }
 
-template <int G, typename AT>
+template <int G, typename AT, bool BN = false>
 __global__ __launch_bounds__(StencilBrick<G>::NTHR, 2) void stencil3_wgrad_kernel(const StencilWArgsT<AT> p) {
   constexpr int C = 16 * G, TZV = StencilBrick<G>::TZV, NTHR = StencilBrick<G>::NTHR, NW = NTHR / 64, NTAPW = (27 + NW - 1) / NW;
   constexpr int HPOSV = (TZV + 2) * HY * HX, NVOXV = TZV * TY * TX;
   __shared__ __attribute__((aligned(16))) __bf16 Xs[HPOSV * C];
   __shared__ __attribute__((aligned(16))) __bf16 Ds[NVOXV * 16];
   __shared__ float bred[NTHR / 16 * 16];
+  __shared__ __attribute__((aligned(16))) float bntab[BN ? 2 * C : 4];
   const int tid = threadIdx.x, lane = tid & 63, wave = tid >> 6;
   const int lr = lane & 15, lg = lane >> 4, q = lr >> 2, pp = lr & 3;
   const int ntap = (27 - wave + NW - 1) / NW;
@@ -277,8 +319,9 @@
     for (int gg = 0; gg < G; ++gg) acc[i][gg] = (f32x4){0.f, 0.f, 0.f, 0.f};
   float bsum = 0.f;
 
-  HaloRegs<G, AT, TZV, NTHR> hr;
+  HaloRegs<G, AT, TZV, NTHR, BN> hr;
   hr.init(p.ldx, p.x_plane, p.cin_load, p.H, p.W, tid);
+  if constexpr (BN) hr.init_bn(p.bn, bntab, p.ldx, p.x_plane, p.cin_load, tid);
   typename V4<AT>::type dr[4];
   auto load_dy = [&](const TileId& t) {
 #pragma unroll
@@ -501,19 +544,26 @@
   return SV_OK;
 }
 
-#define SV_STENCIL_LAUNCH(GG, NTT, VV)                                                                                     \
+#define SV_STENCIL_LAUNCH(GG, NTT, VV, BB)                                                                                 \
   do {                                                                                                                    \
     constexpr int nthr = StencilBrickF<GG>::NTHR;                                                                         \
     const int nt_ = I * (D / StencilBrickF<GG>::TZV) * (H / TY) * (W / TX);                                               \
     a.ntiles = nt_;                                                                                                       \
-    const int resident = 256 * resident_per_cu((const void*)stencil3_fwd_kernel<GG, NTT, AT, VV>, nthr);                  \
-    hipLaunchKernelGGL((stencil3_fwd_kernel<GG, NTT, AT, VV>), dim3(nt_ < resident ? nt_ : resident), dim3(nthr), 0, s, a); \
+    const int resident = 256 * resident_per_cu((const void*)stencil3_fwd_kernel<GG, NTT, AT, VV, BB>, nthr);              \
+    hipLaunchKernelGGL((stencil3_fwd_kernel<GG, NTT, AT, VV, BB>), dim3(nt_ < resident ? nt_ : resident), dim3(nthr), 0, s, a); \
   } while (0)
 
-extern "C" int sv_stencil3_fwd(const void* x, int ldx, int cin_load, int groups, const void* w_bf16, int ntiles16,
-                               const float* bias, void* out, int ldc, int col_off, int cout, const void* residual, int ldr,
-                               double* stats, int I, int D, int H, int W, long long x_plane_stride, long long out_plane_stride,
-                               int act_dtype, void* stream) {
+static int halo_bn_check(const char* who, const float* bn_tab, int tab_ld, int act, int ldx, int cin_load, long long x_plane_stride) {
+  SV_REQUIRE(bn_tab && ((uintptr_t)bn_tab & 15) == 0 && tab_ld % 4 == 0 && tab_ld >= (x_plane_stride ? ldx : cin_load),
+             "%s: bad scale/shift table (tab_ld=%d)", who, tab_ld);
+  SV_REQUIRE(act == SV_ACT_NONE || act == SV_ACT_RELU || act == SV_ACT_LRELU, "%s: activation %d is not supported in the loader", who, act);
+  return SV_OK;
+}
+
+static int stencil3_fwd_impl(const void* x, int ldx, int cin_load, int groups, const void* w_bf16, int ntiles16,
+                             const float* bias, void* out, int ldc, int col_off, int cout, const void* residual, int ldr,
+                             double* stats, int I, int D, int H, int W, long long x_plane_stride, long long out_plane_stride,
+                             const HaloBn* bn, int act_dtype, void* stream) {
   SV_REQUIRE(x && w_bf16 && out, "stencil3_fwd: null argument");
   SV_REQUIRE(x_plane_stride >= 0 && out_plane_stride >= 0 && x_plane_stride % 4 == 0 && out_plane_stride % 4 == 0, "stencil3_fwd: bad plane strides");
   SV_REQUIRE(!out_plane_stride || (col_off == 0 && !residual && ldc % 4 == 0 && cout % ldc == 0),
@@ -534,22 +584,46 @@
     set_error("stencil3_fwd: unsupported (groups=%d, ntiles16=%d)", groups, ntiles16);
     return SV_ERR_INVALID;
   }
+  SV_REQUIRE(!bn || ntiles16 == 1, "stencil3_fwd_bn: a single 16-column tile only (the forward direction)");
   SV_DISPATCH_ACT(act_dtype,
     const int cs4 = (cout + 3) & ~3;
     const bool vec = out_plane_stride != 0 || ((ldc & 3) == 0 && (col_off & 3) == 0 && col_off + cs4 <= ldc && (!residual || ((ldr & 3) == 0 && cs4 <= ldr)));
     StencilArgsT<AT> a{static_cast<const AT*>(x), ldx, cin_load, x_plane_stride, out_plane_stride, (const __bf16*)w_bf16, bias, static_cast<AT*>(out), ldc, col_off, cout,
                        static_cast<const AT*>(residual), ldr, stats, I, D, H, W, ntiles};
-    if (groups == 1 && ntiles16 == 1) { if (vec) SV_STENCIL_LAUNCH(1, 1, true); else SV_STENCIL_LAUNCH(1, 1, false); }
-    else if (groups == 3) { if (vec) SV_STENCIL_LAUNCH(3, 1, true); else SV_STENCIL_LAUNCH(3, 1, false); }
-    else { if (vec) SV_STENCIL_LAUNCH(1, 3, true); else SV_STENCIL_LAUNCH(1, 3, false); });
+    if (bn) {
+      a.bn = *bn;
+      if (groups == 1) { if (vec) SV_STENCIL_LAUNCH(1, 1, true, true); else SV_STENCIL_LAUNCH(1, 1, false, true); }
+      else { if (vec) SV_STENCIL_LAUNCH(3, 1, true, true); else SV_STENCIL_LAUNCH(3, 1, false, true); }
+    }
+    else if (groups == 1 && ntiles16 == 1) { if (vec) SV_STENCIL_LAUNCH(1, 1, true, false); else SV_STENCIL_LAUNCH(1, 1, false, false); }
+    else if (groups == 3) { if (vec) SV_STENCIL_LAUNCH(3, 1, true, false); else SV_STENCIL_LAUNCH(3, 1, false, false); }
+    else { if (vec) SV_STENCIL_LAUNCH(1, 3, true, false); else SV_STENCIL_LAUNCH(1, 3, false, false); });
   return check_launch("sv_stencil3_fwd");
 }
 
+extern "C" int sv_stencil3_fwd(const void* x, int ldx, int cin_load, int groups, const void* w_bf16, int ntiles16,
+                               const float* bias, void* out, int ldc, int col_off, int cout, const void* residual, int ldr,
+                               double* stats, int I, int D, int H, int W, long long x_plane_stride, long long out_plane_stride,
+                               int act_dtype, void* stream) {
+  return stencil3_fwd_impl(x, ldx, cin_load, groups, w_bf16, ntiles16, bias, out, ldc, col_off, cout, residual, ldr, stats, I, D, H, W,
+                           x_plane_stride, out_plane_stride, nullptr, act_dtype, stream);
+}
+
+extern "C" int sv_stencil3_fwd_bn(const void* x, int ldx, int cin_load, int groups, const void* w_bf16, int ntiles16,
+                                  const float* bias, void* out, int ldc, int col_off, int cout, const void* residual, int ldr,
+                                  double* stats, int I, int D, int H, int W, long long x_plane_stride, long long out_plane_stride,
+                                  const float* bn_tab, int tab_ld, int act, float slope, int act_dtype, void* stream) {
+  if (int rc = halo_bn_check("stencil3_fwd_bn", bn_tab, tab_ld, act, ldx, cin_load, x_plane_stride)) return rc;
+  const HaloBn bn{bn_tab, tab_ld, act, slope};
+  return stencil3_fwd_impl(x, ldx, cin_load, groups, w_bf16, ntiles16, bias, out, ldc, col_off, cout, residual, ldr, stats, I, D, H, W,
+                           x_plane_stride, out_plane_stride, &bn, act_dtype, stream);
+}
+
 extern "C" size_t sv_stencil3_wgrad_workspace_floats(int cout, int cin) { return (size_t)WG_SLOTS * cout * cin * 27; }
 
-extern "C" int sv_stencil3_wgrad(const void* x, int ldx, int cin_load, int groups, const void* dy, int lddy, int cout_load,
-                                 float* dw, float* dbias, float* workspace, int cout, int cin, int c_stride, int c_valid, int I, int D, int H,
-                                 int W, long long x_plane_stride, int act_dtype, void* stream) {
+static int stencil3_wgrad_impl(const void* x, int ldx, int cin_load, int groups, const void* dy, int lddy, int cout_load,
+                               float* dw, float* dbias, float* workspace, int cout, int cin, int c_stride, int c_valid, int I, int D, int H,
+                               int W, long long x_plane_stride, const HaloBn* bn, int act_dtype, void* stream) {
   SV_REQUIRE(x && dy && dw, "stencil3_wgrad: null argument");
   SV_REQUIRE(x_plane_stride >= 0 && x_plane_stride % 4 == 0 && (!x_plane_stride || cin_load % ldx == 0), "stencil3_wgrad: bad plane stride");
   SV_REQUIRE_ACT(act_dtype);
@@ -562,16 +636,39 @@
     const int ntiles = I * (D / (groups == 3 ? StencilBrick<3>::TZV : StencilBrick<1>::TZV)) * (H / TY) * (W / TX);
   hipStream_t s = (hipStream_t)stream;
   SV_DISPATCH_ACT(act_dtype,
-    const int per_cu = groups == 1 ? resident_per_cu((const void*)stencil3_wgrad_kernel<1, AT>, StencilBrick<1>::NTHR)
-                                   : resident_per_cu((const void*)stencil3_wgrad_kernel<3, AT>, StencilBrick<3>::NTHR);
+    const void* kern = bn ? (groups == 1 ? (const void*)stencil3_wgrad_kernel<1, AT, true> : (const void*)stencil3_wgrad_kernel<3, AT, true>)
+                          : (groups == 1 ? (const void*)stencil3_wgrad_kernel<1, AT> : (const void*)stencil3_wgrad_kernel<3, AT>);
+    const int per_cu = resident_per_cu(kern, groups == 1 ? StencilBrick<1>::NTHR : StencilBrick<3>::NTHR);
     const int resident = 256 * per_cu;
     const int blocks = ntiles < resident ? ntiles : resident;
     StencilWArgsT<AT> a{static_cast<const AT*>(x), ldx, cin_load, x_plane_stride, static_cast<const AT*>(dy), lddy, cout_load, dw, workspace, dbias, cout, cin, c_stride, c_valid,
                         I, D, H, W, ntiles};
-    if (groups == 1) hipLaunchKernelGGL((stencil3_wgrad_kernel<1, AT>), dim3(blocks), dim3(StencilBrick<1>::NTHR), 0, s, a);
+    if (bn) {
+      a.bn = *bn;
+      if (groups == 1) hipLaunchKernelGGL((stencil3_wgrad_kernel<1, AT, true>), dim3(blocks), dim3(StencilBrick<1>::NTHR), 0, s, a);
+      else hipLaunchKernelGGL((stencil3_wgrad_kernel<3, AT, true>), dim3(blocks), dim3(StencilBrick<3>::NTHR), 0, s, a);
+    }
+    else if (groups == 1) hipLaunchKernelGGL((stencil3_wgrad_kernel<1, AT>), dim3(blocks), dim3(StencilBrick<1>::NTHR), 0, s, a);
     else hipLaunchKernelGGL((stencil3_wgrad_kernel<3, AT>), dim3(blocks), dim3(StencilBrick<3>::NTHR), 0, s, a););
   if (workspace) hipLaunchKernelGGL(stencil_wgrad_fold_kernel, dim3(cdiv(cout * cin * 27, 256)), dim3(256), 0, s, workspace, dw, cout * cin * 27);
   return check_launch("sv_stencil3_wgrad");
+}
+
+extern "C" int sv_stencil3_wgrad(const void* x, int ldx, int cin_load, int groups, const void* dy, int lddy, int cout_load,
+                                 float* dw, float* dbias, float* workspace, int cout, int cin, int c_stride, int c_valid, int I, int D, int H,
+                                 int W, long long x_plane_stride, int act_dtype, void* stream) {
+  return stencil3_wgrad_impl(x, ldx, cin_load, groups, dy, lddy, cout_load, dw, dbias, workspace, cout, cin, c_stride, c_valid, I, D, H, W,
+                             x_plane_stride, nullptr, act_dtype, stream);
+}
+
+extern "C" int sv_stencil3_wgrad_bn(const void* x, int ldx, int cin_load, int groups, const void* dy, int lddy, int cout_load,
+                                    float* dw, float* dbias, float* workspace, int cout, int cin, int c_stride, int c_valid, int I, int D, int H,
+                                    int W, long long x_plane_stride, const float* bn_tab, int tab_ld, int act, float slope, int act_dtype,
+                                    void* stream) {
+  if (int rc = halo_bn_check("stencil3_wgrad_bn", bn_tab, tab_ld, act, ldx, cin_load, x_plane_stride)) return rc;
+  const HaloBn bn{bn_tab, tab_ld, act, slope};
+  return stencil3_wgrad_impl(x, ldx, cin_load, groups, dy, lddy, cout_load, dw, dbias, workspace, cout, cin, c_stride, c_valid, I, D, H, W,
+                             x_plane_stride, &bn, act_dtype, stream);
 }
 
 extern "C" int sv_tconv4s2_fwd(const void* x, const void* w_packed, const float* bias, void* out, double* stats, int I, int D, int H, int W,
diff --git a/swinvox_amd/hip.py b/swinvox_amd/hip.py
--- a/swinvox_amd/hip.py
+++ b/swinvox_amd/hip.py
@@ -38,8 +38,8 @@
 
 _P, _I, _L, _F, _U, _D = C.c_void_p, C.c_int, C.c_longlong, C.c_float, C.c_uint32, C.c_double
 _ACT_TYPED = {
-    "sv_conv_gather", "sv_tconv_gather", "sv_conv_wgrad", "sv_stencil3_fwd", "sv_stencil3_wgrad", "sv_colsum",
-    "sv_layernorm_fwd", "sv_layernorm_bwd", "sv_ln_image_fwd", "sv_ln_image_bwd", "sv_bn_stats", "sv_scale_shift_act", "sv_bn_bwd", "sv_scale_shift_act_signs", "sv_bn_bwd_signs",
+    "sv_conv_gather", "sv_tconv_gather", "sv_conv_wgrad", "sv_stencil3_fwd", "sv_stencil3_wgrad", "sv_stencil3_fwd_bn", "sv_stencil3_wgrad_bn", "sv_colsum",
+    "sv_layernorm_fwd", "sv_layernorm_bwd", "sv_ln_image_fwd", "sv_ln_image_bwd", "sv_bn_stats", "sv_scale_shift_act", "sv_bn_bwd", "sv_scale_shift_act_signs", "sv_bn_bwd_signs", "sv_scale_shift_act_signs_res",
     "sv_window_attention_fwd", "sv_window_attention_bwd", "sv_cross_view_attention_fwd", "sv_cross_view_attention_bwd",
     "sv_transpose", "sv_add_n", "sv_axpby", "sv_relu_bwd", "sv_maxpool2d_fwd", "sv_maxpool2d_bwd", "sv_avgpool2_fwd", "sv_avgpool2_bwd",
     "sv_decoder_seed_fwd", "sv_decoder_seed_bwd", "sv_maxpool3d_fwd", "sv_maxpool3d_bwd", "sv_dropout", "sv_rowscale",
@@ -68,6 +68,8 @@
     "sv_stencil3_fwd": (_I, [_P, _I, _I, _I, _P, _I, _P, _P, _I, _I, _I, _P, _I, _P, _I, _I, _I, _I, _L, _L]),
     "sv_stencil3_wgrad_workspace_floats": (C.c_size_t, None, [_I, _I]),
     "sv_stencil3_wgrad": (_I, [_P, _I, _I, _I, _P, _I, _I, _P, _P, _P, _I, _I, _I, _I, _I, _I, _I, _I, _L]),
+    "sv_stencil3_fwd_bn": (_I, [_P, _I, _I, _I, _P, _I, _P, _P, _I, _I, _I, _P, _I, _P, _I, _I, _I, _I, _L, _L, _P, _I, _I, _F]),
+    "sv_stencil3_wgrad_bn": (_I, [_P, _I, _I, _I, _P, _I, _I, _P, _P, _P, _I, _I, _I, _I, _I, _I, _I, _I, _L, _P, _I, _I, _F]),
     "sv_tconv4s2_fwd": (_I, [_P, _P, _P, _P, _P, _I, _I, _I, _I, _I, _I]),
     "sv_pack_weight": (_I, [_P, _P, _I, _I, _I, _I, _I, _I]),
     "sv_pack_weights_block_elems": (_I, None),
@@ -87,6 +89,7 @@
     "sv_bn_bwd": (_I, [_P, _I, _P, _I, _P, _I, _P, _P, _P, _L, _I, _I, _F, _I, _P, _I, _P, _I, _P, _P, _P, _P, _P]),
     "sv_bn_signs_supported": (_I, None, [_I]),
     "sv_scale_shift_act_signs": (_I, [_P, _I, _P, _P, _P, _I, _P, _I, _L, _I, _I, _F, _P]),
+    "sv_scale_shift_act_signs_res": (_I, [_P, _I, _P, _P, _P, _I, _P, _P, _P, _I, _L, _I, _I, _F, _P]),
     "sv_bn_bwd_signs": (_I, [_P, _I, _P, _P, _I, _P, _P, _P, _L, _I, _I, _F, _I, _P, _I, _P, _I, _P, _P, _P]),
     "sv_window_attention_fwd": (_I, [_P, _P, _P, _I, _I, _I, _I, _I, _I, _I]),
     "sv_window_attention_bwd_workspace_floats": (C.c_size_t, None, [_I]),
diff --git a/swinvox_amd/models/_base.py b/swinvox_amd/models/_base.py
--- a/swinvox_amd/models/_base.py
+++ b/swinvox_amd/models/_base.py
@@ -143,7 +143,18 @@
     def __init__(self, conv: nn.Module, bn: nn.Module, spec: ConvSpec, act: int, slope: float = 0.0):
         self.conv, self.bn, self.spec, self.act, self.slope = conv, bn, spec, act, slope
 
-    def forward(self, x, n, in_grid, training, *, ldi=None, z=None, ldz=None, residual=None, ldr=0):
+    def forward_raw(self, x, n, in_grid, training, *, ldi=None):
+        sp = self.spec
+        assert self.act == ACT_NONE
+        og = sp.out_grid(in_grid)
+        M = n * og[0] * og[1] * og[2]
+        y = empty(M, sp.cout, like=x)
+        st = BatchNormState(self.bn, M, training)
+        sp.forward(x, n, in_grid, self._pack("f"), y, ldi=ldi, bias=self.conv.bias, stats=st.sums)
+        st.finalize()
+        return y, og, (x, ldi, y, None, sp.cout, st, n, in_grid, M)
+
+    def forward(self, x, n, in_grid, training, *, ldi=None, z=None, ldz=None, residual=None, ldr=0, res_bn=None):
         sp = self.spec
         og = sp.out_grid(in_grid)
         M = n * og[0] * og[1] * og[2]
@@ -154,7 +165,7 @@
         st.finalize()
         if z is None:
             z, ldz = empty(M, sp.cout, like=x), sp.cout
-        st.apply(y, sp.cout, z, ldz, self.act, self.slope, residual, ldr)
+        st.apply(y, sp.cout, z, ldz, self.act, self.slope, residual, ldr, res_bn=res_bn)
         return z, og, (x, ldi, y, z if residual is not None else None, ldz, st, n, in_grid, M)
 
     def backward(self, ctx, dz, lddz, grads, *, need_dx=True, dres=None, lddres=0, dx=None, lddx=None, dx_epi=None):
diff --git a/swinvox_amd/models/encoder.py b/swinvox_amd/models/encoder.py
--- a/swinvox_amd/models/encoder.py
+++ b/swinvox_amd/models/encoder.py
@@ -35,10 +35,15 @@
     def fwd(self, x, n, grid, training):
         a, g1, c1 = self._c1.forward(x, n, grid, training)
         b, g2, c2 = self._c2.forward(a, n, g1, training)
-        idt, cd = x, None
+        idt, cd, st_d = x, None, None
+        Co = self.conv3.out_channels
         if self._cd is not None:
-            idt, _, cd = self._cd.forward(x, n, grid, training)
-        out, g3, c3 = self._c3.forward(b, n, g2, training, residual=idt, ldr=self.conv3.out_channels)
+            if training and ops._bn_signs_on() and ops.bn_fold_skip_enabled() and Co % 256 == 0:
+                idt, _, cd = self._cd.forward_raw(x, n, grid, training)
+                st_d = cd[5]
+            else:
+                idt, _, cd = self._cd.forward(x, n, grid, training)
+        out, g3, c3 = self._c3.forward(b, n, g2, training, residual=idt, ldr=Co, res_bn=st_d)
         return out, g3, (c1, c2, c3, cd)
 
     def bwd(self, ctx, dout, grads):
diff --git a/swinvox_amd/models/merger.py b/swinvox_amd/models/merger.py
--- a/swinvox_amd/models/merger.py
+++ b/swinvox_amd/models/merger.py
@@ -53,11 +53,15 @@
         call("sv_merger_pack", ptr(w), ptr(wp), w.shape[0], w.shape[1], 1 if dgrad else 0, 1 if li == 4 else 0)
         return wp
 
-    def _conv_fwd(self, li, x, ldi, y, ldc, stats, w5p=None):
+    def _conv_fwd(self, li, x, ldi, y, ldc, stats, w5p=None, bn_tab=None):
         conv, I = self._layer(li)[0], y.shape[0] // VOX
         if ops.get_math() == "bf16":
-            call("sv_stencil3_fwd", ptr(x), ldi, 48 if li == 4 else 12, 3 if li == 4 else 1, ptr(self._stencil_pack(li, False)), 1,
-                 ptr(conv.bias), ptr(y), ldc, 0, conv.out_channels, None, 0, ptr(stats), I, 32, 32, 32, I * VOX * 12 if li == 4 else 0, 0)
+            args = (ptr(x), ldi, 48 if li == 4 else 12, 3 if li == 4 else 1, ptr(self._stencil_pack(li, False)), 1,
+                    ptr(conv.bias), ptr(y), ldc, 0, conv.out_channels, None, 0, ptr(stats), I, 32, 32, 32, I * VOX * 12 if li == 4 else 0, 0)
+            if bn_tab is not None:
+                call("sv_stencil3_fwd_bn", *args, ptr(bn_tab), 12, ACT_LRELU, self._slope)
+            else:
+                call("sv_stencil3_fwd", *args)
         else:
             sp = self._spec(li)
             sp.forward(x, I, G, sp.pack_fwd(w5p if li == 4 else conv.weight), y, ldi=ldi, ldc=ldc, bias=conv.bias, stats=stats)
@@ -73,13 +77,17 @@
             epi = dict(residual=dx, ldr=lddx) if accumulate else {}
             sp.dgrad(dy, I, G, sp.pack_dgrad(w5p if li == 4 else conv.weight), dx, lddy=lddy, lddx=lddx, **epi)
 
-    def _conv_wgrad(self, li, dy, lddy, x, ldx, grads):
+    def _conv_wgrad(self, li, dy, lddy, x, ldx, grads, bn_tab=None):
         conv, I = self._layer(li)[0], dy.shape[0] // VOX
         if ops.get_math() == "bf16":
             ws = ops.zeros_f64(8 * conv.out_channels * conv.in_channels * 27, dy.device)
-            call("sv_stencil3_wgrad", ptr(x), ldx, 48 if li == 4 else 12, 3 if li == 4 else 1, ptr(dy), lddy, lddy if lddy <= 12 else 12,
-                 ptr(grads[conv.weight]), ptr(grads[conv.bias]), ptr(ws), conv.out_channels, conv.in_channels, 12 if li == 4 else 16, 9, I, 32, 32, 32,
-                 I * VOX * 12 if li == 4 else 0)
+            args = (ptr(x), ldx, 48 if li == 4 else 12, 3 if li == 4 else 1, ptr(dy), lddy, lddy if lddy <= 12 else 12,
+                    ptr(grads[conv.weight]), ptr(grads[conv.bias]), ptr(ws), conv.out_channels, conv.in_channels, 12 if li == 4 else 16, 9, I, 32, 32, 32,
+                    I * VOX * 12 if li == 4 else 0)
+            if bn_tab is not None:
+                call("sv_stencil3_wgrad_bn", *args, ptr(bn_tab), 12, ACT_LRELU, self._slope)
+            else:
+                call("sv_stencil3_wgrad", *args)
         elif li == 4:
             dw5p = fzeros(9, 48, 27, like=dy)
             self._s5.wgrad(dy, x, I, G, dw5p, lddy=lddy, ldx=ldx, async_ok=False)
@@ -98,6 +106,11 @@
         x12 = ops.to_store(as_channels_last12(raw))
         vol = ops.to_store(vol)
         planar = ops.get_math() == "bf16"
+        fold = planar and ops.bn_fold_stencil_enabled()
+        tab = None
+        if fold:
+            t64 = ops.zeros_f64(61, vol.device)
+            tab = (t64[1:] if t64.data_ptr() % 16 else t64[:60]).view(torch.float32).view(5, 2, 12)
         buf = empty if planar else zeros
         cat = empty(4, M, 12, like=vol) if planar else zeros(M, 48, like=vol)
         ldz = 12 if planar else 48
@@ -105,6 +118,15 @@
         ctx14, xin, ldi = [], x12, 12
         for k in range(4):
             bn = self._layer(k)[1]
+            if fold:
+                y = cat[k]
+                st = BatchNormState(bn, M, tr, scale_shift=(tab[k, 0, :9], tab[k, 1, :9]))
+                self._conv_fwd(k, xin, ldi, y, 12, st.sums, bn_tab=tab[k - 1] if k else None)
+                st.finalize()
+                st.probe(y, 12)
+                ctx14.append((xin, ldi, y, None, st))
+                xin, ldi = y, 12
+                continue
             y = empty(M, 12, like=vol)
             st = BatchNormState(bn, M, tr)
             self._conv_fwd(k, xin, ldi, y, 12, st.sums)
@@ -114,24 +136,29 @@
             ctx14.append((xin, ldi, y, z, st))
             xin, ldi = z, ldz
         y5 = empty(M, 12, like=vol)
-        st5 = BatchNormState(self.layer5[1], M, tr)
-        self._conv_fwd(4, cat, ldz, y5, 12, st5.sums, w5p)
+        st5 = BatchNormState(self.layer5[1], M, tr, scale_shift=(tab[4, 0, :9], tab[4, 1, :9]) if fold else None)
+        self._conv_fwd(4, cat, ldz, y5, 12, st5.sums, w5p, bn_tab=tab[:4] if fold else None)
         st5.finalize()
-        z5 = buf(M, 12, like=vol)
-        st5.apply(y5, 12, z5, 12, ACT_LRELU, sl)
+        if fold:
+            st5.probe(y5, 12)
+            z5 = None
+        else:
+            z5 = buf(M, 12, like=vol)
+            st5.apply(y5, 12, z5, 12, ACT_LRELU, sl)
         y6 = empty(M, 1, like=vol)
         st6 = BatchNormState(self.layer6[1], M, tr)
-        self._conv_fwd(5, z5, 12, y6, 1, st6.sums)
+        self._conv_fwd(5, y5 if fold else z5, 12, y6, 1, st6.sums, bn_tab=tab[4] if fold else None)
         st6.finalize()
         wl = empty(M, 1, like=vol)
         st6.apply(y6, 1, wl, 1, ACT_LRELU, sl)
         out = empty(B, 32, 32, 32, like=vol)
         call("sv_merge_views_fwd", ptr(wl), ptr(vol), ptr(out), B, V, VOX)
-        tape = (B, V, x12, vol, cat, ctx14, w5p, y5, st5, z5, y6, st6, wl, out, raw_dtype, vol_dtype) if save else None
+        tape = (B, V, x12, vol, cat, ctx14, w5p, y5, st5, z5, y6, st6, wl, out, raw_dtype, vol_dtype, tab) if save else None
         return ops.to_f32(out), tape
 
     def _bwd(self, tape, grads, in_needs, dout):
-        B, V, x12, vol, cat, ctx14, w5p, y5, st5, z5, y6, st6, wl, out, raw_dtype, vol_dtype = tape
+        B, V, x12, vol, cat, ctx14, w5p, y5, st5, z5, y6, st6, wl, out, raw_dtype, vol_dtype, tab = tape
+        fold = tab is not None
         M, sl = B * V * VOX, self._slope
         dout = ops.to_store(dout)
         dwl = empty(M, 1, like=vol)
@@ -141,7 +168,7 @@
         dy6 = zeros(M, 4, like=vol)
         st6.backward(dwl, 1, None, 0, y6, 1, dy6, 4, grads[bn6.weight], grads[bn6.bias], ACT_LRELU, sl)
         self._bias_grad(dy6, M, 1, 4, grads[conv6.bias])
-        self._conv_wgrad(5, dy6, 4, z5, 12, grads)
+        self._conv_wgrad(5, dy6, 4, y5 if fold else z5, 12, grads, bn_tab=tab[4] if fold else None)
         buf = empty if ops.get_math() == "bf16" else zeros
         dz5 = buf(M, 12, like=vol)
         self._conv_dgrad(5, dy6, 4, dz5, 12, False)
@@ -151,7 +178,7 @@
         self._bias_grad(dy5, M, 9, 12, grads[conv5.bias])
         planar = cat.dim() == 3
         ldz = 12 if planar else 48
-        self._conv_wgrad(4, dy5, 12, cat, ldz, grads)
+        self._conv_wgrad(4, dy5, 12, cat, ldz, grads, bn_tab=tab[:4] if fold else None)
         dcat = empty(4, M, 12, like=vol) if planar else zeros(M, 48, like=vol)
         self._conv_dgrad(4, dy5, 12, dcat, ldz, False, w5p)
         dx = None
@@ -162,7 +189,7 @@
             dy = buf(M, 12, like=vol)
             st.backward(dzk, ldz, None, 0, y, 12, dy, 12, grads[bn.weight], grads[bn.bias], ACT_LRELU, sl)
             self._bias_grad(dy, M, 9, 12, grads[conv.bias])
-            self._conv_wgrad(k, dy, 12, xin, ldi, grads)
+            self._conv_wgrad(k, dy, 12, xin, ldi, grads, bn_tab=tab[k - 1] if fold and k else None)
             if k > 0:
                 self._conv_dgrad(k, dy, 12, dcat[k - 1] if planar else dcat[:, 12 * (k - 1):], ldz, True)
             else:
diff --git a/swinvox_amd/ops.py b/swinvox_amd/ops.py
--- a/swinvox_amd/ops.py
+++ b/swinvox_amd/ops.py
@@ -599,12 +599,14 @@
 
 class BatchNormState:
 
-    def __init__(self, bn: torch.nn.Module, M: int, training: bool):
+    def __init__(self, bn: torch.nn.Module, M: int, training: bool, scale_shift=None):
         self.bn, self.M, self.training, self.C = bn, M, training, bn.num_features
         dev = bn.weight.device
         self.sums = zeros_f64(BN_SLOTS * 2 * self.C, dev) if training else None
         buf = fempty(4 * self.C, device=dev)
         self.scale, self.shift, self.mean, self.rstd = buf[:self.C], buf[self.C:2 * self.C], buf[2 * self.C:3 * self.C], buf[3 * self.C:]
+        if scale_shift is not None:
+            self.scale, self.shift = scale_shift
 
     def finalize(self):
         bn = self.bn
@@ -621,15 +623,22 @@
         if probe is not None:
             probe(self, x, ldx)
 
-    def apply(self, x, ldx, y, ldy, act=ACT_NONE, slope=0.0, residual=None, ldr=0):
+    def apply(self, x, ldx, y, ldy, act=ACT_NONE, slope=0.0, residual=None, ldr=0, res_bn=None):
         self.probe(x, ldx)
         self.signs = None
         if (residual is not None and act != ACT_NONE and self.training and _bn_signs_on() and self.C % 256 == 0
                 and self.C % 4 == 0 and ldx % 4 == 0 and ldy % 4 == 0 and ldr % 4 == 0):
             self.signs = torch.empty(self.M * (self.C // 64), dtype=torch.int64, device=x.device)
+            if res_bn is not None:
+                res_bn.probe(residual, ldr)
+                call("sv_scale_shift_act_signs_res", ptr(x), ldx, ptr(self.scale), ptr(self.shift), ptr(residual), ldr, ptr(res_bn.scale),
+                     ptr(res_bn.shift), ptr(y), ldy, self.M, self.C, act, slope, ptr(self.signs))
+                return
             call("sv_scale_shift_act_signs", ptr(x), ldx, ptr(self.scale), ptr(self.shift), ptr(residual), ldr, ptr(y), ldy, self.M, self.C, act, slope,
                  ptr(self.signs))
             return
+        if res_bn is not None:
+            raise RuntimeError("BatchNormState.apply: res_bn needs the sign-word pass")
         call("sv_scale_shift_act", ptr(x), ldx, ptr(self.scale), ptr(self.shift), ptr(residual), ldr, ptr(y), ldy, self.M, self.C, act, slope)
 
     def backward(self, dz, lddz, z, ldz, x, ldx, dx, lddx, dgamma, dbeta, act=ACT_NONE, slope=0.0, dres=None, lddres=0):
@@ -652,6 +661,24 @@
     _STATE["bn_signs"] = bool(on)
 
 
+def bn_fold_skip_enabled() -> bool:
+    import os
+    return _STATE.get("bn_fold_skip", os.environ.get("SV_BN_FOLD_SKIP", "1") != "0")
+
+
+def set_bn_fold_skip(on: bool) -> None:
+    _STATE["bn_fold_skip"] = bool(on)
+
+
+def bn_fold_stencil_enabled() -> bool:
+    import os
+    return _STATE.get("bn_fold_stencil", os.environ.get("SV_BN_FOLD_STENCIL", "1") != "0")
+
+
+def set_bn_fold_stencil(on: bool) -> None:
+    _STATE["bn_fold_stencil"] = bool(on)
+
+
 def input_prep_enabled() -> bool:
     import os
     return _STATE.get("input_prep", os.environ.get("SV_INPUT_PREP", "1") != "0")
```

Result: no change. 4766 views/s (-0.8%).
